# balisujohn/tortoise.cpp

Hardware: AMD Instinct MI355X
Metric: audio-seconds/sec end-to-end (AR+diffusion+vocoder), 16 cands x 80 steps (higher is better)
Workload: dtype f16 MFMA inputs / f32 accumulate (diffusion, vocoder convs); f32 weights, f16 KV (AR)

## Files before the change

### include/tortoise_mi355x.h

```cpp
#ifndef TORTOISE_MI355X_H
#define TORTOISE_MI355X_H

#include <stdint.h>

#ifdef __cplusplus
extern "C" {
#endif

typedef struct tts_ctx tts_ctx;

typedef enum {
  TTS_OK = 0,
  TTS_ERR_ARG = -1,
  TTS_ERR_IO = -2,
  TTS_ERR_FORMAT = -3,
  TTS_ERR_HIP = -4,
  TTS_ERR_STATE = -5,
  TTS_ERR_LIMIT = -6
} tts_status;

enum { TTS_VOCAB_MEL = 8194, TTS_DMODEL = 1024, TTS_MEL_CH = 100, TTS_CODES = 502 };

#define TTS_API_VERSION 8
int tts_version(void);
// ... 78 lines not shown
int tts_cvvp_latent_dim(const tts_ctx *ctx);
int tts_cvvp_rows(int mel_frames);
int tts_cvvp_voice(tts_ctx *ctx, const float *mel80, const int32_t *frames, int n_clips, float *latents_out);
int tts_cvvp_voice_audio(tts_ctx *ctx, const float *audio, const int64_t *n_samples, const int32_t *sample_rate, int n_clips, const tts_voice_audio_opts *opts,
                         float *latents_out);
int tts_cvvp_score(tts_ctx *ctx, const float *voice_latents, int n_clips, const int32_t *codes, const int32_t *code_len, int n_candidates, int code_stride,
                   float *scores_out);

int tts_diffusion_frames(int latent_rows);

int tts_load_hifigan(tts_ctx *ctx, const char *path);
int tts_hifigan_samples(int latent_rows);
#define TTS_HFG_HALO_FRAMES 24
int tts_hifigan_decode(tts_ctx *ctx, const float *latents, const int32_t *rows, int n_candidates, const float *voices, int n_voices,
                       const int32_t *voice_of_candidate, float *audio_out);
int tts_hifigan_chunk(tts_ctx *ctx, const float *latents, const int32_t *rows, int n_candidates, const float *voices, int n_voices,
                      const int32_t *voice_of_candidate, const int32_t *frame0, const int32_t *n_frames, float *audio_out);
typedef int (*tts_audio_cb)(void *user, const float *samples, int n_samples, int is_last);
int tts_hifigan_stream(tts_ctx *ctx, const int32_t *text_ids, int n_text, const float *voice1024, int max_steps, unsigned flags, int stride_codes,
                       tts_audio_cb cb, void *user, int32_t *codes_out , int32_t *rows_out, float *latents_out , int32_t *steps_out);
int tts_hifigan_stream_recaptures(const tts_ctx *ctx);
int tts_ar_session_open(tts_ctx *ctx, int n_slots, int max_cand, int max_text, int max_steps, unsigned flags);
int tts_ar_session_admit(tts_ctx *ctx, const int32_t *text_ids, int n_text, const float *voice1024, int n_cand, uint32_t seed,
                         const int32_t *stop_at );
int tts_ar_session_room(const tts_ctx *ctx);
int tts_ar_session_step(tts_ctx *ctx);
int tts_ar_session_finished(tts_ctx *ctx, int32_t *ids_out, int cap);
int tts_ar_session_collect(tts_ctx *ctx, int request, int32_t *codes_out , int32_t *rows_out, float *latents_out ,
                           int32_t *steps_out, int32_t *stopped_out );
int tts_ar_session_logits(tts_ctx *ctx, int request, float *logits_out );
int tts_ar_session_cancel(tts_ctx *ctx, int request);
int tts_ar_session_close(tts_ctx *ctx);
int tts_ar_session_recaptures(const tts_ctx *ctx);
int tts_ar_session_enable_audio(tts_ctx *ctx, int stride_steps);
int tts_ar_session_audio(tts_ctx *ctx, int request, float *out, int cap_samples, int32_t *is_last);
enum { TTS_AR_ROW_CONTROLS = 8 };
typedef struct tts_ar_request {
  uint32_t struct_size;
  int32_t n_cand;
  uint32_t seed;
  int32_t max_steps;
  const int32_t *stop_at;
  double temperature, top_k, top_p, repetition_penalty, penalty_scope;
  double typical_mass;
} tts_ar_request;
int tts_ar_request_init(tts_ctx *ctx, tts_ar_request *req);
int tts_ar_session_admit_ex(tts_ctx *ctx, const int32_t *text_ids, int n_text, const float *voice1024, const tts_ar_request *req);
int tts_host_ar_request_check(const tts_ar_request *req, int max_cand, int max_steps);
int tts_host_session_first_fit(const uint8_t *busy, int n_slots, int n_cand);
typedef struct tts_diff_request {
  uint32_t struct_size;
  int32_t n_cand;
  const float *latents;
  const int32_t *rows;
  const float *voice_latent2048;
  int32_t n_steps;
  int32_t sampler;
  double ddim_eta, cond_free_k;
  const float *noise;
  uint32_t seed;
  double temperature;
  int32_t cond_free;
} tts_diff_request;
int tts_diff_request_init(tts_ctx *ctx, tts_diff_request *req);
int tts_diff_session_open(tts_ctx *ctx, int max_packed_rows, int max_requests);
int tts_diff_session_admit(tts_ctx *ctx, const tts_diff_request *req);
int tts_diff_session_room(const tts_ctx *ctx);
int tts_diff_session_step(tts_ctx *ctx);
int tts_diff_session_finished(tts_ctx *ctx, int32_t *ids, int cap);
int tts_diff_session_collect(tts_ctx *ctx, int request, float *mel_out);
int tts_diff_session_cancel(tts_ctx *ctx, int request);
int tts_diff_session_close(tts_ctx *ctx);
int tts_diff_session_captures(const tts_ctx *ctx);
int tts_host_diff_packed_rows(const int32_t *latent_rows, int n_cand);
int tts_host_diff_packed_rows_ex(const int32_t *latent_rows, int n_cand, int cond_free);
int tts_host_diff_request_check(const tts_diff_request *req, int max_packed_rows);
int tts_diffusion_forward(tts_ctx *ctx, const float *latents, int latent_rows, const float *x_t,
                          int timestep, int conditioning_free, float *out);
enum { TTS_NOISE_REFERENCE = 0, TTS_NOISE_DEVICE = 1 };
int tts_diffusion(tts_ctx *ctx, const float *latents, const int32_t *rows, int n_candidates,
                  int n_steps, const float *noise, int noise_mode, float *mel_out);
int tts_diffusion_last_layout(const tts_ctx *ctx, int32_t *packed_rows_out, int32_t *sequences_out);
int tts_diffusion_time_mlp_retries(const tts_ctx *ctx);
int tts_diffusion_fp16_check(tts_ctx *ctx, int64_t counts[2]);

int tts_vocoder_samples(int mel_frames);
int tts_vocoder(tts_ctx *ctx, const float *mel, const int32_t *frames, int n_candidates,
                const float *noise, int noise_mode, float *audio_out);

int tts_vocoder_chunk(tts_ctx *ctx, const float *mel, int mel_frames, const float *noise, int frame0, int n_frames,
                      float *audio_out, int *n_samples_out);

int tts_load_bigvgan(tts_ctx *ctx, const char *path);
int tts_bigvgan_samples(int mel_frames);
int tts_bigvgan(tts_ctx *ctx, const float *mel, const int32_t *frames, int n_candidates, float *audio_out);
int tts_bigvgan_config(tts_ctx *ctx, int32_t out[8]);

#define TTS_CLS_MAX_SAMPLES 220000
int tts_load_classifier(tts_ctx *ctx, const char *path);
int tts_classifier_positions(int n_samples_24k);
int tts_classify_audio(tts_ctx *ctx, const float *audio, const int64_t *n_samples, const int32_t *sample_rate, int n_clips, float *prob_out,
                       float *logits_out);

int tts_load_aligner(tts_ctx *ctx, const char *path);
int tts_aligner_frames(int n_samples_16k);
int tts_aligner_clip_frames(tts_ctx *ctx, int64_t n_samples, int sample_rate);
int tts_aligner_vocab(tts_ctx *ctx, int32_t *vocab_out, int cap, int32_t *blank_out);
int tts_aligner_ids(tts_ctx *ctx, const float *audio, const int64_t *n_samples, const int32_t *sample_rate, int n_clips, int32_t *ids_out,
                    int32_t *n_frames_out, int frame_stride, float *logits_out);
int tts_align_audio(tts_ctx *ctx, const float *audio, int64_t n_samples, int sample_rate, const char *text, int64_t *offsets_out, int cap);
int64_t tts_redact_audio(tts_ctx *ctx, const float *audio, int64_t n_samples, int sample_rate, const char *text, float *out, int64_t cap);
int tts_host_ctc_decode(const int32_t *ids, int n_frames, const int32_t *vocab, int n_vocab, int blank, char *out, int cap);
int tts_host_max_alignment(const char *s1, const char *s2, char *out, int cap);
int tts_host_ctc_align(const int32_t *ids, int n_frames, const int32_t *vocab, int n_vocab, int blank, const char *text, int64_t n_samples,
                       int64_t *offsets_out, int cap);
int tts_host_redact_spans(const char *text, char *clean_out, int cap, int32_t *intervals_out, int cap_intervals);

#define TTS_RANDOM_VOICE_MAX 4096
enum { TTS_RANDOM_VOICE_AUTO = 0, TTS_RANDOM_VOICE_DIFFUSION = 1 };
int tts_load_random_voice(tts_ctx *ctx, const char *auto_path, const char *diff_path);
int tts_random_voice_dim(const tts_ctx *ctx, int side);
int tts_random_voice(tts_ctx *ctx, const uint64_t *seeds, int n, const float *z_auto, const float *z_diff, float *out_auto, float *out_diff);
int tts_random_voice_noise(tts_ctx *ctx, uint64_t seed, int side, float *out, int cap);
int tts_host_blend_voices(const float *latents, const float *weights, int n, int dim, float *out);
int tts_host_random_voice_fold(const float *w, const float *b, int dim, int equal, float *w_out, float *b_out);

#define TTS_DVAE_MAX_CLIPS 256
#define TTS_DVAE_MAX_FRAMES 16384
int tts_load_dvae(tts_ctx *ctx, const char *path);
int tts_dvae_rows(int mel_frames);
int tts_dvae_tokens(const tts_ctx *ctx);
int tts_dvae_dim(const tts_ctx *ctx);
int tts_dvae_codes(tts_ctx *ctx, const float *mel80, const int32_t *frames, int n_clips, int32_t *codes_out, int32_t *n_codes_out, int code_stride,
                   float *z_out);
int tts_dvae_codes_audio(tts_ctx *ctx, const float *audio, const int64_t *n_samples, const int32_t *sample_rate, int n_clips,
                         const tts_voice_audio_opts *opts, int32_t *codes_out, int32_t *n_codes_out, int code_stride, float *z_out);
int tts_ar_latents_for_codes(tts_ctx *ctx, const int32_t *text_ids, int n_text, const float *voice1024, const int32_t *codes, int n_codes,
                             int32_t *rows_out, float *latents_out);

#define TTS_SCORE_POS_DECODE 0
#define TTS_SCORE_POS_TRAIN 1
int tts_ar_score_codes(tts_ctx *ctx, const int32_t *text_ids, int n_text, const float *voice1024, const int32_t *codes, const int32_t *n_codes, int n_cand,
                       int code_stride, int positions, float *logp_out, float *stop_logp_out, int32_t *greedy_out, float *lse_out);
int tts_host_ar_score_rows(const int32_t *codes, int n_codes, int positions, int32_t *input_ids, int32_t *mel_pos, int32_t *targets);

int tts_write_wav(const char *path, const float *samples, int64_t n, int sample_rate);

int tts_host_schedule_ddim(int n_steps, double eta, double *acp, double *acp_prev, float *c_x0, float *c_eps, float *sigma);
int tts_host_schedule_dpmpp(int n_steps, float *a, float *b, float *c, int32_t *order);
int tts_host_schedule(int n_steps, int32_t *timestep_map, float *max_log, float *min_log, float *cfk, float *sqrt_recip,
                      float *sqrt_recipm1, float *coef1, float *coef2);
void tts_host_timestep_embedding(int t, float *out1024);
int tts_host_rel_bucket(int query, int key);
int tts_host_sample_row(const float *row8194, const int32_t *penalty_ids, int n_ids, float uniform);
int tts_host_sample_prefiltered(const float *row8194, const int32_t *penalty_ids, int n_ids, float uniform, int keep);
int tts_host_sample_row_ex(const float *row8194, const int32_t *penalty_ids, int n_ids, float uniform, float temperature, int top_k, float top_p, float penalty,
                           int mode);
int tts_host_sample_prefiltered_ex(const float *row8194, const int32_t *penalty_ids, int n_ids, float uniform, float temperature, int top_k, float top_p,
                                   float penalty, int keep, int already_penalised);
int tts_host_typical_keep(const float *row8194, double mass, uint8_t *keep_out8194);
int tts_host_sample_row_typical(const float *row8194, const int32_t *penalty_ids, int n_ids, float uniform, float temperature, int top_k, float top_p,
                                float penalty, double typical_mass, int mode);
int tts_host_sample_prefiltered_typical(const float *row8194, const int32_t *penalty_ids, int n_ids, float uniform, float temperature, int top_k, float top_p,
                                        float penalty, double typical_mass, int keep);
int tts_host_pad_codes(const int32_t *codes, int n, int32_t *out502);
int tts_host_stream_final_rows(const int32_t *codes, int k);
// ... 16 lines not shown
```

### tortoise.cpp_amd/__init__.py

```python
import ctypes as C
import os
import subprocess
import numpy as np

HERE = os.path.dirname(os.path.abspath(__file__))
LIB_PATH = os.environ.get("TTS_LIB_PATH") or os.path.join(HERE, "libtortoise_mi355x.so")
HEADER = os.path.join(os.path.dirname(HERE), "include", "tortoise_mi355x.h")
VOCAB_MEL = 8194
DMODEL = 1024
AR_MASK_STOP = 1
AR_RETIRE = 2
AR_ROW_CONTROLS = 8
NOISE_REFERENCE, NOISE_DEVICE = 0, 1
SAMPLER_DDPM, SAMPLER_DDIM, SAMPLER_DPMPP_2M = 0, 1, 3
SCORE_POSITIONS = {"decode": 0, "train": 1}

_f32p = np.ctypeslib.ndpointer(np.float32, flags="C_CONTIGUOUS")
_i32p = np.ctypeslib.ndpointer(np.int32, flags="C_CONTIGUOUS")
_f64p = np.ctypeslib.ndpointer(np.float64, flags="C_CONTIGUOUS")
AUDIO_CB = C.CFUNCTYPE(C.c_int, C.c_void_p, C.POINTER(C.c_float), C.c_int, C.c_int)


def build(verbose=False):
    subprocess.check_call(["make", "-C", HERE, "-j8", "all"], stdout=None if verbose else subprocess.DEVNULL)


class ArRequest(C.Structure):
    _fields_ = [("struct_size", C.c_uint32), ("n_cand", C.c_int32), ("seed", C.c_uint32), ("max_steps", C.c_int32), ("stop_at", C.c_void_p),
                ("temperature", C.c_double), ("top_k", C.c_double), ("top_p", C.c_double), ("repetition_penalty", C.c_double), ("penalty_scope", C.c_double),
                ("typical_mass", C.c_double)]


AR_REQUEST_SIZE_V0 = ArRequest.typical_mass.offset


class DiffRequest(C.Structure):
    _fields_ = [("struct_size", C.c_uint32), ("n_cand", C.c_int32), ("latents", C.c_void_p), ("rows", C.c_void_p), ("voice_latent2048", C.c_void_p),
                ("n_steps", C.c_int32), ("sampler", C.c_int32), ("ddim_eta", C.c_double), ("cond_free_k", C.c_double), ("noise", C.c_void_p), ("seed", C.c_uint32),
                ("temperature", C.c_double), ("cond_free", C.c_int32)]


class VoiceAudioOpts(C.Structure):
    _fields_ = [("struct_size", C.c_uint32), ("mel_norms80", C.c_void_p), ("crop_offset", C.c_int64), ("full_clips", C.c_int32)]


AR_CONTROL_FIELDS = {"temperature": "temperature", "top_k": "top_k", "top_p": "top_p", "penalty": "repetition_penalty", "scope": "penalty_scope",
                     "typical_mass": "typical_mass"}


class TtsError(RuntimeError):
    pass


_lib = None


def lib():
    global _lib
    if _lib is not None:
        return _lib
    if not os.path.exists(LIB_PATH):
        raise TtsError("libtortoise_mi355x.so is not built (run __graft_entry__.build()); there is no fallback path")
    L = C.CDLL(LIB_PATH)
    vp, ci, cf = C.c_void_p, C.c_int, C.c_float
    sig = {
        "tts_version": (ci, []), "tts_create": (vp, [ci]), "tts_destroy": (None, [vp]), "tts_last_error": (C.c_char_p, [vp]),
        "tts_set_option": (ci, [vp, C.c_char_p, C.c_double]),
        "tts_load_ar": (ci, [vp, C.c_char_p]), "tts_load_diffusion": (ci, [vp, C.c_char_p]),
        "tts_load_vocoder": (ci, [vp, C.c_char_p]), "tts_load_clvp": (ci, [vp, C.c_char_p]),
        "tts_load_diffusion_conditioning_encoder": (ci, [vp, C.c_char_p]), "tts_diffusion_conditioning_latent": (ci, [vp, _f32p, _i32p, ci, _f32p]),
        "tts_set_diffusion_conditioning_latent": (ci, [vp, _f32p]),
        "tts_load_voice_encoder": (ci, [vp, C.c_char_p]), "tts_voice_latent": (ci, [vp, _f32p, _i32p, ci, _f32p]),
        "tts_load_cvvp": (ci, [vp, C.c_char_p]), "tts_cvvp_latent_dim": (ci, [vp]), "tts_cvvp_rows": (ci, [ci]),
        "tts_cvvp_voice": (ci, [vp, vp, vp, ci, vp]), "tts_cvvp_voice_audio": (ci, [vp, vp, vp, vp, ci, vp, vp]),
        "tts_cvvp_score": (ci, [vp, vp, ci, vp, vp, ci, ci, vp]),
        "tts_clvp_score": (ci, [vp, _i32p, ci, _i32p, _i32p, ci, ci, _f32p]), "tts_ar_layers": (ci, [vp]), "tts_diffusion_layers": (ci, [vp]),
        "tts_seed": (None, [vp, C.c_uint32]), "tts_rng_load_state": (ci, [vp, C.c_char_p]), "tts_rng_save_state": (ci, [vp, C.c_char_p]),
        "tts_rng_uniform": (cf, [vp]), "tts_rng_normal": (None, [vp, _f32p, C.c_int64]),
        "tts_tokenizer_load": (ci, [vp, C.c_char_p]), "tts_tokenize": (ci, [vp, C.c_char_p, _i32p, ci]),
        "tts_ar_begin": (ci, [vp, _i32p, ci, _f32p, ci, ci]), "tts_ar_prefill": (ci, [vp, _f32p]),
        "tts_ar_step": (ci, [vp, _i32p, ci, _f32p]), "tts_ar_latents": (ci, [vp, _i32p, ci, ci, _f32p]),
        "tts_sample": (ci, [vp, _f32p, _i32p, ci, ci, _i32p]),
        "tts_ar_step_sample": (ci, [vp, _i32p, ci, C.c_uint, _i32p]), "tts_ar_topk_fallbacks": (ci, [vp]), "tts_diffusion_time_mlp_retries": (ci, [vp]), "tts_diffusion_fp16_check": (ci, [vp, C.POINTER(C.c_int64)]),
        "tts_device_numa_node": (ci, [vp, C.c_char_p, ci]), "tts_pin_to_device_numa_node": (ci, [vp]),
        "tts_host_sample_row": (ci, [_f32p, _i32p, ci, cf]), "tts_host_sample_prefiltered": (ci, [_f32p, _i32p, ci, cf, ci]),
        "tts_host_sample_row_ex": (ci, [_f32p, _i32p, ci, cf, cf, ci, cf, cf, ci]), "tts_host_sample_prefiltered_ex": (ci, [_f32p, _i32p, ci, cf, cf, ci, cf, cf, ci, ci]),
        "tts_host_typical_keep": (ci, [_f32p, C.c_double, vp]),
        "tts_host_sample_row_typical": (ci, [_f32p, _i32p, ci, cf, cf, ci, cf, cf, C.c_double, ci]),
        "tts_host_sample_prefiltered_typical": (ci, [_f32p, _i32p, ci, cf, cf, ci, cf, cf, C.c_double, ci]),
        "tts_autoregressive": (ci, [vp, _i32p, ci, _f32p, ci, ci, C.c_uint, _i32p, _i32p, vp, _i32p]),
        "tts_ar_stop_status": (ci, [vp, _i32p, ci]), "tts_ar_set_stop_schedule": (ci, [vp, C.c_void_p, ci]),
        "tts_ar_begin_multi": (ci, [vp, _i32p, _i32p, ci, _f32p, _i32p, ci]),
        "tts_autoregressive_multi": (ci, [vp, _i32p, _i32p, ci, _f32p, _i32p, ci, C.c_uint, _i32p, _i32p, vp, _i32p]),
        "tts_split_text": (ci, [vp, C.c_char_p, ci, _i32p, _i32p, ci]),
        "tts_ar_begin_multi_voice": (ci, [vp, _i32p, _i32p, ci, vp, ci, vp, _i32p, ci]),
        "tts_autoregressive_multi_voice": (ci, [vp, _i32p, _i32p, ci, vp, ci, vp, _i32p, ci, C.c_uint, _i32p, _i32p, vp, _i32p]),
        "tts_diffusion_multi_voice": (ci, [vp, _f32p, _i32p, ci, vp, ci, vp, ci, vp, ci, _f32p]),
        "tts_split_turns": (ci, [vp, C.c_char_p, ci, ci, _i32p, _i32p, _i32p, ci]),
        "tts_host_ar_stop_run": (ci, [_i32p, ci, _i32p, ci, C.c_uint, vp, _i32p, _i32p, _i32p, vp]),
        "tts_diffusion_frames": (ci, [ci]),
        "tts_load_hifigan": (ci, [vp, C.c_char_p]), "tts_hifigan_samples": (ci, [ci]),
        "tts_hifigan_decode": (ci, [vp, vp, vp, ci, vp, ci, vp, vp]),
        "tts_hifigan_chunk": (ci, [vp, vp, vp, ci, vp, ci, vp, vp, vp, vp]),
        "tts_load_bigvgan": (ci, [vp, C.c_char_p]), "tts_bigvgan_samples": (ci, [ci]), "tts_bigvgan": (ci, [vp, vp, vp, ci, vp]),
        "tts_bigvgan_config": (ci, [vp, vp]),
        "tts_load_classifier": (ci, [vp, C.c_char_p]), "tts_classifier_positions": (ci, [ci]), "tts_classify_audio": (ci, [vp, vp, vp, vp, ci, vp, vp]),
        "tts_load_aligner": (ci, [vp, C.c_char_p]), "tts_aligner_frames": (ci, [ci]), "tts_aligner_clip_frames": (ci, [vp, C.c_int64, ci]),
        "tts_aligner_vocab": (ci, [vp, vp, ci, vp]), "tts_aligner_ids": (ci, [vp, vp, vp, vp, ci, vp, vp, ci, vp]),
        "tts_align_audio": (ci, [vp, vp, C.c_int64, ci, C.c_char_p, vp, ci]), "tts_redact_audio": (C.c_int64, [vp, vp, C.c_int64, ci, C.c_char_p, vp, C.c_int64]),
        "tts_host_ctc_decode": (ci, [vp, ci, vp, ci, ci, vp, ci]), "tts_host_max_alignment": (ci, [C.c_char_p, C.c_char_p, vp, ci]),
        "tts_host_ctc_align": (ci, [vp, ci, vp, ci, ci, C.c_char_p, C.c_int64, vp, ci]), "tts_host_redact_spans": (ci, [C.c_char_p, vp, ci, vp, ci]),
        "tts_load_random_voice": (ci, [vp, C.c_char_p, C.c_char_p]), "tts_random_voice_dim": (ci, [vp, ci]),
        "tts_random_voice": (ci, [vp, vp, ci, vp, vp, vp, vp]), "tts_random_voice_noise": (ci, [vp, C.c_uint64, ci, vp, ci]),
        "tts_load_dvae": (ci, [vp, C.c_char_p]), "tts_dvae_rows": (ci, [ci]), "tts_dvae_tokens": (ci, [vp]), "tts_dvae_dim": (ci, [vp]),
        "tts_dvae_codes": (ci, [vp, vp, vp, ci, vp, vp, ci, vp]), "tts_dvae_codes_audio": (ci, [vp, vp, vp, vp, ci, vp, vp, vp, ci, vp]),
        "tts_ar_latents_for_codes": (ci, [vp, vp, ci, vp, vp, ci, vp, vp]),
        "tts_ar_score_codes": (ci, [vp, vp, ci, vp, vp, vp, ci, ci, ci, vp, vp, vp, vp]), "tts_host_ar_score_rows": (ci, [vp, ci, ci, vp, vp, vp]),
        "tts_host_blend_voices": (ci, [vp, vp, ci, ci, vp]), "tts_host_random_voice_fold": (ci, [vp, vp, ci, ci, vp, vp]),
        "tts_hifigan_stream": (ci, [vp, vp, ci, vp, ci, C.c_uint, ci, vp, vp, vp, vp, vp, vp]), "tts_hifigan_stream_recaptures": (ci, [vp]),
        "tts_host_stream_final_rows": (ci, [vp, ci]),
        "tts_ar_session_open": (ci, [vp, ci, ci, ci, ci, C.c_uint]), "tts_ar_session_admit": (ci, [vp, vp, ci, vp, ci, C.c_uint32, vp]),
        "tts_ar_session_room": (ci, [vp]), "tts_ar_session_step": (ci, [vp]), "tts_ar_session_finished": (ci, [vp, vp, ci]),
        "tts_ar_session_collect": (ci, [vp, ci, vp, vp, vp, vp, vp]), "tts_ar_session_logits": (ci, [vp, ci, vp]),
        "tts_ar_session_cancel": (ci, [vp, ci]), "tts_ar_session_close": (ci, [vp]), "tts_ar_session_recaptures": (ci, [vp]),
        "tts_ar_session_enable_audio": (ci, [vp, ci]), "tts_ar_session_audio": (ci, [vp, ci, vp, ci, vp]),
        "tts_host_session_first_fit": (ci, [vp, ci, ci]),
        "tts_ar_request_init": (ci, [vp, C.POINTER(ArRequest)]), "tts_ar_session_admit_ex": (ci, [vp, vp, ci, vp, C.POINTER(ArRequest)]),
        "tts_host_ar_request_check": (ci, [C.POINTER(ArRequest), ci, ci]),
        "tts_diff_request_init": (ci, [vp, C.POINTER(DiffRequest)]), "tts_diff_session_open": (ci, [vp, ci, ci]),
        "tts_diff_session_admit": (ci, [vp, C.POINTER(DiffRequest)]), "tts_diff_session_room": (ci, [vp]), "tts_diff_session_step": (ci, [vp]),
        "tts_diff_session_finished": (ci, [vp, vp, ci]), "tts_diff_session_collect": (ci, [vp, ci, vp]), "tts_diff_session_cancel": (ci, [vp, ci]),
        "tts_diff_session_close": (ci, [vp]), "tts_diff_session_captures": (ci, [vp]),
        "tts_host_diff_packed_rows": (ci, [vp, ci]), "tts_host_diff_packed_rows_ex": (ci, [vp, ci, ci]),
        "tts_diffusion_last_layout": (ci, [vp, _i32p, _i32p]), "tts_host_diff_request_check": (ci, [C.POINTER(DiffRequest), ci]),
        "tts_diffusion_forward": (ci, [vp, _f32p, ci, _f32p, ci, ci, _f32p]),
        "tts_diffusion": (ci, [vp, _f32p, _i32p, ci, ci, vp, ci, _f32p]),
        "tts_vocoder_samples": (ci, [ci]),
        "tts_vocoder": (ci, [vp, _f32p, _i32p, ci, vp, ci, _f32p]),
        "tts_vocoder_chunk": (ci, [vp, _f32p, ci, _f32p, ci, ci, _f32p, C.POINTER(ci)]),
        "tts_write_wav": (ci, [C.c_char_p, _f32p, C.c_int64, ci]), "tts_read_wav": (C.c_int64, [C.c_char_p, vp, C.c_int64, vp]),
        "tts_voice_audio_opts_init": (ci, [C.POINTER(VoiceAudioOpts)]),
        "tts_voice_from_audio": (ci, [vp, vp, vp, vp, ci, vp, vp, vp]), "tts_audio_mel": (ci, [vp, vp, C.c_int64, ci, ci, vp, vp, C.c_int64]),
        "tts_host_schedule": (ci, [ci, _i32p] + [_f32p] * 7), "tts_host_schedule_ddim": (ci, [ci, C.c_double, _f64p, _f64p, _f32p, _f32p, _f32p]),
        "tts_host_schedule_dpmpp": (ci, [ci, _f32p, _f32p, _f32p, _i32p]), "tts_host_timestep_embedding": (None, [ci, _f32p]),
        "tts_host_rel_bucket": (ci, [ci, ci]), "tts_host_pad_codes": (ci, [_i32p, ci, _i32p]), "tts_host_trimmed_rows": (ci, [_i32p]),
        "tts_host_fp8_e4m3": (C.c_uint8, [cf]), "tts_host_mel_frames": (ci, [C.c_int64]),
        "tts_host_mel_diffusion100": (ci, [_f32p, C.c_int64, ci, _f32p]), "tts_host_mel_voice80": (ci, [_f32p, C.c_int64, vp, _f32p]),
        "tts_prof_reset": (ci, [vp, ci]), "tts_prof_get": (ci, [vp, C.c_char_p, C.POINTER(C.c_double), C.POINTER(C.c_int64), C.POINTER(C.c_double)]),
    }
    for name, (res, args) in sig.items():
        fn = getattr(L, name)
        fn.restype = res
        fn.argtypes = args
    _lib = L
    return L


def header_symbols():
    import re
    txt = open(HEADER).read()
    txt = re.sub(r"/\*.*?\*/", "", txt, flags=re.S)
    return sorted(set(re.findall(r"\b(tts_[a-z0-9_]+)\s*\(", txt)))


def _ptr(a):
    return None if a is None else a.ctypes.data_as(C.c_void_p)
# ... 34 lines not shown
    def set_option(self, key, value):
        self._ck(self.L.tts_set_option(self.h, key.encode(), float(value)))

    def load(self, model_dir=None, ar=None, diffusion=None, vocoder=None):
        if model_dir:
            ar = ar or os.path.join(model_dir, "ggml-model.bin")
            diffusion = diffusion or os.path.join(model_dir, "ggml-diffusion-model.bin")
            vocoder = vocoder or os.path.join(model_dir, "ggml-vocoder-model.bin")
        if ar:
            self._ck(self.L.tts_load_ar(self.h, ar.encode()))
        if diffusion:
            self._ck(self.L.tts_load_diffusion(self.h, diffusion.encode()))
        if vocoder:
            self._ck(self.L.tts_load_vocoder(self.h, vocoder.encode()))

    @property
    def ar_layers(self):
        return self.L.tts_ar_layers(self.h)

    def seed(self, s):
        self.L.tts_seed(self.h, s)

    def rng_load_state(self, path):
        self._ck(self.L.tts_rng_load_state(self.h, path.encode()))

    def rng_save_state(self, path):
        self._ck(self.L.tts_rng_save_state(self.h, path.encode()))

    def rng_uniform(self):
        return self.L.tts_rng_uniform(self.h)

    def rng_normal(self, n):
        out = np.empty(n, np.float32)
        self.L.tts_rng_normal(self.h, out, n)
        return out

    def tokenizer_load(self, path):
        return self._ck(self.L.tts_tokenizer_load(self.h, path.encode()))

    def tokenize(self, message):
        out = np.empty(4096, np.int32)
        n = self._ck(self.L.tts_tokenize(self.h, message.encode("utf-8"), out, 4096))
        return out[:n].copy()

    def ar_begin(self, tokens, voice, B, max_steps):
        self.B = B
        self._ck(self.L.tts_ar_begin(self.h, np.ascontiguousarray(tokens, np.int32), len(tokens),
                                     np.ascontiguousarray(voice, np.float32), B, max_steps))

    def ar_prefill(self):
        out = np.empty((self.B, VOCAB_MEL), np.float32)
        self._ck(self.L.tts_ar_prefill(self.h, out.reshape(-1)))
        return out

    def ar_step(self, prev_ids, i):
        out = np.empty((self.B, VOCAB_MEL), np.float32)
        self._ck(self.L.tts_ar_step(self.h, np.ascontiguousarray(prev_ids, np.int32), i, out.reshape(-1)))
        return out

    def ar_step_sample(self, prev_ids, i, mask_stop=False):
        out = np.empty(self.B, np.int32)
        self._ck(self.L.tts_ar_step_sample(self.h, np.ascontiguousarray(prev_ids, np.int32), i, 1 if mask_stop else 0, out))
        return out

    def topk_fallbacks(self):
        return self.L.tts_ar_topk_fallbacks(self.h)

    def numa_node(self):
        buf = C.create_string_buffer(1024)
        node = self.L.tts_device_numa_node(self.h, buf, 1024)
        return node, buf.value.decode()

    def pin_to_numa_node(self):
        return self.L.tts_pin_to_device_numa_node(self.h)

    def fp16_check(self):
        c = (C.c_int64 * 2)()
        self._ck(self.L.tts_diffusion_fp16_check(self.h, c))
        return int(c[0]), int(c[1])

    def time_mlp_retries(self):
        return self.L.tts_diffusion_time_mlp_retries(self.h)

    def ar_latents(self, codes502, n_mel=502):
        codes502 = np.ascontiguousarray(codes502, np.int32).reshape(-1, 502)
        nb = codes502.shape[0]
        out = np.empty((nb, min(500, n_mel), DMODEL), np.float32)
        self._ck(self.L.tts_ar_latents(self.h, codes502.reshape(-1), nb, n_mel, out.reshape(-1)))
        return out

    def sample(self, logits, penalty_ids):
        logits = np.ascontiguousarray(logits, np.float32)
        ids = np.ascontiguousarray(penalty_ids, np.int32).reshape(logits.shape[0], -1)
        out = np.empty(logits.shape[0], np.int32)
        self._ck(self.L.tts_sample(self.h, logits.reshape(-1), ids.reshape(-1), ids.shape[1], logits.shape[0], out))
        return out

    def set_stop_schedule(self, stop_at=None):
        if stop_at is None:
            self._ck(self.L.tts_ar_set_stop_schedule(self.h, None, 0))
        else:
            a = np.ascontiguousarray(stop_at, np.int32)
            self._ck(self.L.tts_ar_set_stop_schedule(self.h, a.ctypes.data_as(C.c_void_p), len(a)))

    def autoregressive(self, tokens, voice, B, max_steps, mask_stop=False, want_latents=True, retire=False):
        codes = np.empty((B, 502), np.int32)
        rows = np.empty(B, np.int32)
        steps = np.zeros(1, np.int32)
        lat = np.empty((B * 500, DMODEL), np.float32) if want_latents else None
        self._ck(self.L.tts_autoregressive(self.h, np.ascontiguousarray(tokens, np.int32), len(tokens),
                                           np.ascontiguousarray(voice, np.float32), B, max_steps,
                                           (AR_MASK_STOP if mask_stop else 0) | (AR_RETIRE if retire else 0), codes.reshape(-1), rows, _ptr(lat), steps))
        lats = None
        if want_latents:
            lats, off = [], 0
            for r in rows:
                lats.append(lat[off:off + r].copy())
                off += r
        return codes, rows, lats, int(steps[0])

    def ar_begin_multi(self, prompts, voice=None, n_cand=1, max_steps=1, voices=None, voice_of_prompt=None):
        ids, lens, nc = _prompt_args(prompts, n_cand)
        self.B = int(nc.sum())
        if voices is None and voice_of_prompt is None:
            self._ck(self.L.tts_ar_begin_multi(self.h, ids, lens, len(lens), np.ascontiguousarray(voice, np.float32), nc, max_steps))
            return
        tab, nv, idx = _voice_args(voice, voices, voice_of_prompt, DMODEL)
        self._ck(self.L.tts_ar_begin_multi_voice(self.h, ids, lens, len(lens), _ptr(tab), nv, _ptr(idx), nc, max_steps))

    def autoregressive_multi(self, prompts, voice=None, n_cand=1, max_steps=1, mask_stop=False, retire=False, want_latents=True, voices=None, voice_of_prompt=None):
        ids, lens, nc = _prompt_args(prompts, n_cand)
        B = int(nc.sum())
        codes = np.empty((B, 502), np.int32)
        rows = np.empty(B, np.int32)
        steps = np.zeros(1, np.int32)
        lat = np.empty((B * 500, DMODEL), np.float32) if want_latents else None
        flags = (AR_MASK_STOP if mask_stop else 0) | (AR_RETIRE if retire else 0)
        if voices is None and voice_of_prompt is None:
            self._ck(self.L.tts_autoregressive_multi(self.h, ids, lens, len(lens), np.ascontiguousarray(voice, np.float32), nc, max_steps, flags,
                                                     codes.reshape(-1), rows, _ptr(lat), steps))
        else:
            tab, nv, idx = _voice_args(voice, voices, voice_of_prompt, DMODEL)
            self._ck(self.L.tts_autoregressive_multi_voice(self.h, ids, lens, len(lens), _ptr(tab), nv, _ptr(idx), nc, max_steps, flags, codes.reshape(-1), rows,
                                                           _ptr(lat), steps))
        c0 = np.concatenate([[0], np.cumsum(nc)])
        out_codes = [codes[c0[g]:c0[g + 1]].copy() for g in range(len(nc))]
        out_rows = [rows[c0[g]:c0[g + 1]].copy() for g in range(len(nc))]
        out_lats = None
        if want_latents:
            out_lats, off = [], 0
            for g in range(len(nc)):
                lg = []
                for r in out_rows[g]:
                    lg.append(lat[off:off + r].copy())
                    off += r
                out_lats.append(lg)
        return out_codes, out_rows, out_lats, int(steps[0])

    def split_text(self, message, max_ids):
        raw = message.encode("utf-8")
        cap = len(raw) + 1
        starts, lens = np.empty(cap, np.int32), np.empty(cap, np.int32)
        n = self._ck(self.L.tts_split_text(self.h, raw, max_ids, starts, lens, cap))
        return [raw[starts[k]:starts[k] + lens[k]].decode("utf-8") for k in range(n)]

    def split_turns(self, message, n_voices, max_ids=404):
# ... 868 lines not shown
```

### tortoise.cpp_amd/csrc/api.cpp

```cpp
#include "common.h"
#include <sched.h>
#include <cctype>
#include <cstddef>
#include <cmath>
#include <algorithm>
#include <chrono>
#include <fstream>
#include <new>

using namespace tts;

hipEvent_t tts::prof_event(tts_ctx *c) {
  if (!c->ev_pool.empty()) { hipEvent_t e = c->ev_pool.back(); c->ev_pool.pop_back(); return e; }
  hipEvent_t e = nullptr;
  (void)hipEventCreate(&e);
  return e;
}

template <class F>
static int guarded(tts_ctx *c, F body) {
  try {
    return body();
  } catch (const std::bad_alloc &) {
    return fail(c, TTS_ERR_LIMIT, "out of host memory");
// ... 86 lines not shown
  diff_session_close(c);
  if (c->ar) ar_free(c->ar);
  if (c->diff) diff_free(c->diff);
  if (c->voc) voc_free(c->voc);
  if (c->clvp) clvp_free(c->clvp);
  if (c->cvvp) cvvp_free(c->cvvp);
  if (c->venc) voice_enc_free(c->venc);
  if (c->dcond) diff_cond_enc_free(c->dcond);
  if (c->hifigan) hifigan_free(c->hifigan);
  if (c->bigvgan) bigvgan_free(c->bigvgan);
  if (c->classifier) classifier_free(c->classifier);
  if (c->aligner) aligner_free(c->aligner);
  if (c->dvae) dvae_free(c->dvae);
  if (c->rlg) random_voice_free(c->rlg);
  if (c->afe) afe_free(c->afe);
  if (c->fp16_counts) (void)hipFree(c->fp16_counts);
  delete c->tok;
  for (auto &kv : c->prof)
    for (auto &pr : kv.second.pending) { (void)hipEventDestroy(pr.first); (void)hipEventDestroy(pr.second); }
  for (hipEvent_t e : c->ev_pool) (void)hipEventDestroy(e);
  if (c->ev0) (void)hipEventDestroy(c->ev0);
  if (c->ev1) (void)hipEventDestroy(c->ev1);
  if (c->stream) (void)hipStreamDestroy(c->stream);
  if (c->load_stream) (void)hipStreamDestroy(c->load_stream);
  delete c;
}

int tts_version(void) { return TTS_API_VERSION; }

const char *tts_last_error(const tts_ctx *c) { return c ? c->err.c_str() : "no context (no HIP device?)"; }

static const char *const kArControlKeys[6] = {"ar_temperature", "ar_top_k", "ar_top_p", "ar_repetition_penalty", "ar_penalty_scope", "ar_typical_mass"};
static int ar_control_index(const std::string &k) {
  for (int i = 0; i < 6; i++)
    if (k == kArControlKeys[i]) return i;
  return -1;
}
static const char *ar_control_error(int which, double value) {
  static_assert(TTS_VOCAB_MEL == 8194, "the text below names the vocabulary size");
  switch (which) {
  case 0: return (!std::isfinite(value) || !(value > 0) || !std::isfinite((float)value) || !((float)value > 0)) ? "ar_temperature: a finite value > 0" : nullptr;
  case 1: return (!(value >= 1 && value <= TTS_VOCAB_MEL) || value != std::floor(value)) ? "ar_top_k: an integer in 1 .. 8194" : nullptr;
  case 2: return (!(value > 0 && value <= 1) || !((float)value > 0)) ? "ar_top_p: a value in (0, 1]" : nullptr;
  case 3: return (!std::isfinite(value) || !(value >= 1) || !std::isfinite((float)value)) ? "ar_repetition_penalty: a finite value >= 1" : nullptr;
  case 4: return (value != 0 && value != 1) ? "ar_penalty_scope: 0 (the ids of the last input) or 1 (every id fed since tts_ar_begin)" : nullptr;
  case 5: return (value != 0 && (!(value > 0 && value < 1) || !((float)value > 0 && (float)value < 1))) ? "ar_typical_mass: 0 (off) or a value in (0, 1)" : nullptr;
  }
  return "unknown sampler control";
}
static void ar_control_store(int which, double value, SamplerParams &sp, int &scope) {
  switch (which) {
  case 0: sp.temp = (float)value; break;
  case 1: sp.top_k = (int)value; break;
  case 2: sp.top_p = (float)value; break;
  case 3: sp.penalty = (float)value; break;
  case 4: scope = (int)value; break;
  case 5: sp.typ_mass = (float)value; break;
  }
}

int tts_set_option(tts_ctx *c, const char *key, double value) {
  if (!c || !key) return TTS_ERR_ARG;
  std::string k(key);
  if (k == "gn_eps") c->gn_eps = (float)value;
  else if (k == "ggml_lut") c->ggml_lut = value != 0;
  else if (k.rfind("prof_only:", 0) == 0) {
    if (value != 0) c->prof_filter.push_back(k.substr(10));
    else c->prof_filter.clear();
  }
  else if (k == "device_topk") c->device_topk = value != 0;
  else if (k == "sampler_threads") {
    if (c->sampler_pool) { sampler_pool_free(c->sampler_pool); c->sampler_pool = nullptr; }
    c->sampler_threads = value < 0 ? -1 : (int)value;
  }
  else if (k == "share_uncond") c->share_uncond = value != 0;
  else if (k == "prof_stride") c->prof_stride = value < 1 ? 1 : (int)value;
  else if (k == "diff_graph") c->diff_graph = value != 0;
  else if (k == "dec_f32_mfma") c->dec_f32_mfma = value != 0;
  else if (k == "attn_f32") c->attn_f32 = value != 0;
  else if (k == "attn_proj_f16") c->attn_proj_f16 = value != 0;
  else if (k == "proj_dual_b") c->proj_dual_b = value != 0;
  else if (k == "gemm_wreg") c->gemm_wreg = value == 1 ? tts_ctx::GEMM_WREG_ALL : value == 2 ? 1 : value == 3 ? 2 : value == 4 ? 4 : 0;
  else if (k == "gemm_gn_fuse") c->gemm_gn_fuse = value != 0;
  else if (k == "lc_attn_f32") c->lc_attn_f32 = value != 0;
  else if (k == "latency_mode") c->latency_mode = value != 0;
  else if (k == "fp16_check") c->fp16_check = value != 0;
  else if (k == "rng_fast_normal") c->rng_fast_normal = value != 0;
  else if (k == "noise_pipeline") c->noise_pipeline = value != 0;
  else if (k == "load_device_pack") c->load_device_pack = value != 0;
  else if (k == "load_threads") c->load_threads = value < 0 ? 0 : value > 64 ? 64 : (int)value;
  else if (k == "attn_q64") c->attn_q64 = value < 0 ? 0 : value > 2 ? 2 : (int)value;
  else if (k == "hoist_integrator") c->hoist_integrator = value < 0 ? 0 : (int)value;
  else if (k == "attn_f32_drop") c->attn_f32_drop = (int)value & 7;
  else if (k == "ar_weights") {
    if (value != 0 && value != 1 && value != 2) return fail(c, TTS_ERR_ARG, "ar_weights: 0 (f32), 1 (fp16) or 2 (fp8 e4m3)");
    c->ar_weights = (int)value;
  }
  else if (k == "diff_sampler") {
    if (const char *e = diff_control_error(0, value)) return fail(c, TTS_ERR_ARG, "%s", e);
    c->diff_sampler = (int)value;
  }
  else if (k == "ddim_eta") {
    if (const char *e = diff_control_error(1, value)) return fail(c, TTS_ERR_ARG, "%s", e);
    c->ddim_eta = value;
  }
  else if (k == "cond_free_k") {
    if (const char *e = diff_control_error(2, value)) return fail(c, TTS_ERR_ARG, "%s", e);
    c->cond_free_k = (float)value;
  }
  else if (k == "diff_temperature") {
    if (const char *e = diff_control_error(3, value)) return fail(c, TTS_ERR_ARG, "%s", e);
    c->diff_temperature = value;
  }
  else if (k == "cond_free") {
    if (const char *e = diff_control_error(4, value)) return fail(c, TTS_ERR_ARG, "%s", e);
    c->cond_free = (int)value;
  }
  else if (ar_control_index(k) >= 0) {
    const int which = ar_control_index(k);
    if (const char *e = ar_control_error(which, value)) return fail(c, TTS_ERR_ARG, "%s", e);
    ar_control_store(which, value, c->ar_sp, c->ar_penalty_scope);
  }
  else if (k == "hfg_small_m") {
    if (!(value >= 0 && value <= (1 << 24)) || value != std::floor(value)) return fail(c, TTS_ERR_ARG, "hfg_small_m: a row count in 0 .. 2^24 (0 = never)");
    c->hfg_small_m = (int)value;
  }
  else if (k == "prof_eager_every") c->prof_eager_every = value < 1 ? 1 : (int)value;
  else if (k == "stream_cus") {
    if (c->device < 0) return fail(c, TTS_ERR_HIP, "host-only context: no stream");
    if (c->ar || c->diff || c->voc || c->clvp || c->cvvp || c->venc || c->dcond || c->hifigan) return fail(c, TTS_ERR_STATE, "stream_cus must be set before the models are loaded");
    (void)hipSetDevice(c->device);
    hipDeviceProp_t prop;
    if (hipGetDeviceProperties(&prop, c->device) != hipSuccess) return fail(c, TTS_ERR_HIP, "hipGetDeviceProperties failed");
    const int xcds = 8, per_xcd = prop.multiProcessorCount / xcds, n = (int)(value < 0 ? -value : value);
    if (prop.multiProcessorCount % xcds || per_xcd > 32 || n >= per_xcd) return fail(c, TTS_ERR_ARG, "stream_cus %d: the device has %d CUs per XCD", (int)value, per_xcd);
    hipStream_t s = nullptr;
    if (n == 0) {
      if (hipStreamCreate(&s) != hipSuccess) return fail(c, TTS_ERR_HIP, "hipStreamCreate failed");
    } else {
      uint32_t mask[8] = {0, 0, 0, 0, 0, 0, 0, 0};
      for (int slot = 0; slot < per_xcd; slot++)
        if ((slot < n) == (value > 0))
          for (int x = 0; x < xcds; x++) { const int bit = slot * xcds + x; mask[bit >> 5] |= 1u << (bit & 31); }
      if (hipExtStreamCreateWithCUMask(&s, (uint32_t)((per_xcd * xcds + 31) / 32), mask) != hipSuccess)
        return fail(c, TTS_ERR_HIP, "hipExtStreamCreateWithCUMask failed");
    }
    (void)hipStreamSynchronize(c->stream);
    (void)hipStreamDestroy(c->stream);
    c->stream = s;
    c->stream_cus = (int)value;
  }
  else if (k == "rng_shard_offset") { if (value < 0) return fail(c, TTS_ERR_ARG, "rng_shard_offset < 0"); c->rng_shard_offset = (int)value; }
  else if (k == "rng_shard_total") { if (value < 0) return fail(c, TTS_ERR_ARG, "rng_shard_total < 0"); c->rng_shard_total = (int)value; }
  else return fail(c, TTS_ERR_ARG, "unknown option '%s'", key);
  return TTS_OK;
}

#define NEED_CTX(c)                                                                              \
  do {                                                                                         \
    if (!(c)) return TTS_ERR_ARG;                                                              \
    if ((c)->device < 0) return fail((c), TTS_ERR_HIP, "host-only context: no HIP device, no CPU fallback"); \
    (void)hipSetDevice((c)->device);                                                           \
  } while (0)

#define NO_SESSION(c, name)                                                                                          \
  do {                                                                                                               \
// ... 271 lines not shown
    for (int b = 0; b < n_cand; b++)
      for (int j = 0; j <= n_codes[b]; j++) {
        const size_t r = (size_t)b * n_rows + j;
        if (lse_out) lse_out[b * os + j] = out[r];
        logp_out[b * os + j] = out[R + r];
        if (stop_logp_out) stop_logp_out[b * os + j] = out[2 * R + r];
        if (greedy_out) memcpy(&greedy_out[b * os + j], &out[3 * R + r], 4);
      }
    return TTS_OK;
  });
}
int tts_host_stream_final_rows(const int32_t *codes, int k) { return (k < 0 || (k > 0 && !codes)) ? TTS_ERR_ARG : stream_final_rows(codes, k); }
int tts_ar_layers(const tts_ctx *c) { return c ? ar_layers(c) : 0; }
int tts_diffusion_layers(const tts_ctx *c) { return c ? diff_layers(c) : 0; }

void tts_seed(tts_ctx *c, uint32_t seed) {
  if (!c) return;
  c->seed_value = seed;
  c->generator.seed(seed);
  c->distribution.reset();
  c->normal_distribution.reset();
}
int tts_rng_load_state(tts_ctx *c, const char *path) {
  if (!c) return TTS_ERR_ARG;
  std::ifstream fin(path);
  if (!fin) return fail(c, TTS_ERR_IO, "cannot open '%s'", path);
  fin >> c->generator;
  c->distribution.reset();
  c->normal_distribution.reset();
  return fin ? TTS_OK : fail(c, TTS_ERR_FORMAT, "bad RNG state file '%s'", path);
}
int tts_rng_save_state(tts_ctx *c, const char *path) {
  if (!c || !path) return TTS_ERR_ARG;
  std::ofstream fout(path);
  if (!fout) return fail(c, TTS_ERR_IO, "cannot open '%s' for writing", path);
  fout << c->generator;
  return fout ? TTS_OK : fail(c, TTS_ERR_IO, "cannot write '%s'", path);
}
float tts_rng_uniform(tts_ctx *c) { return c ? c->distribution(c->generator) : 0.f; }
void tts_rng_normal(tts_ctx *c, float *out, int64_t n) {
  if (!c || !out || n <= 0) return;
  rng_normal_fill(c, out, n);
}

int tts_tokenizer_load(tts_ctx *c, const char *path) {
  if (!c || !path) return TTS_ERR_ARG;
  return guarded(c, [&] {
    std::unique_ptr<Tokenizer> t(new Tokenizer());
    if (!t->load(path)) return fail(c, TTS_ERR_IO, "Failed to open %s (missing, truncated or malformed)", path);
    delete c->tok;
    c->tok = t.release();
    return (int)c->tok->vocab.size();
  });
}
int tts_tokenize(tts_ctx *c, const char *message, int32_t *out, int cap) {
  if (!c || !c->tok) return c ? fail(c, TTS_ERR_STATE, "tokenizer not loaded") : TTS_ERR_ARG;
  if (!message || !out || cap < 0) return fail(c, TTS_ERR_ARG, "tts_tokenize: bad argument");
  return guarded(c, [&] {
    std::vector<int> ids = c->tok->encode(message);
    for (int i = 0; i < (int)ids.size() && i < cap; i++) out[i] = ids[i];
    return (int)ids.size();
  });
}

int tts_ar_begin(tts_ctx *c, const int32_t *ids, int n, const float *voice, int B, int max_steps) {
  NEED_CTX(c);
  NO_SESSION(c, "tts_ar_begin");
  return guarded(c, [&] { return ar_begin(c, ids, n, voice, B, max_steps); });
}
int tts_ar_prefill(tts_ctx *c, float *logits) { NEED_CTX(c); NO_SESSION(c, "tts_ar_prefill"); return guarded(c, [&] { return ar_prefill(c, logits); }); }
int tts_ar_step(tts_ctx *c, const int32_t *prev, int i, float *logits) {
  NEED_CTX(c);
  NO_SESSION(c, "tts_ar_step");
  return guarded(c, [&] { return ar_step(c, prev, i, logits, 0); });
}
int tts_ar_step_sample(tts_ctx *c, const int32_t *prev, int i, unsigned flags, int32_t *samples_out) {
  NEED_CTX(c);
  NO_SESSION(c, "tts_ar_step_sample");
  if (!prev || !samples_out) return TTS_ERR_ARG;
  return guarded(c, [&] { return ar_drv_step_sample(c, prev, i, flags, samples_out); });
}
int tts_ar_topk_fallbacks(const tts_ctx *c) { return c ? c->topk_fallbacks : -1; }
int tts_diffusion_time_mlp_retries(const tts_ctx *c) { return c ? c->time_mlp_retries : -1; }
int tts_diffusion_fp16_check(tts_ctx *c, int64_t counts[2]) {
  if (!c || !counts) return TTS_ERR_ARG;
  return guarded(c, [&] { return tts::diff_fp16_check(c, counts); });
}
int tts_host_sample_row(const float *row, const int32_t *ids, int ids_per_cand, float uniform) {
  if (!row || !ids || ids_per_cand < 1) return -1;
  return sample_one_row(row, ids, ids_per_cand, uniform);
}
static bool sampler_params_ok(const float *row, const int32_t *ids, int n_ids, float temperature, int top_k, float top_p, float penalty) {
  if (!row || n_ids < 0 || (n_ids > 0 && !ids)) return false;
  for (int i = 0; i < n_ids; i++)
    if (ids[i] < 0 || ids[i] >= TTS_VOCAB_MEL) return false;
  return std::isfinite(temperature) && temperature > 0 && top_k >= 1 && top_k <= TTS_VOCAB_MEL && top_p > 0 && top_p <= 1 && std::isfinite(penalty) && penalty >= 1;
}
int tts_host_sample_row_ex(const float *row, const int32_t *ids, int n_ids, float uniform, float temperature, int top_k, float top_p, float penalty, int mode) {
  if (!sampler_params_ok(row, ids, n_ids, temperature, top_k, top_p, penalty) || (mode != 0 && mode != 1)) return -2;
  SamplerParams sp; sp.temp = temperature; sp.top_k = top_k; sp.top_p = top_p; sp.penalty = penalty;
  return sample_one_row_ex(row, ids, n_ids, uniform, sp, mode == 1);
}
int tts_host_sample_prefiltered_ex(const float *row, const int32_t *ids, int n_ids, float uniform, float temperature, int top_k, float top_p, float penalty, int keep,
                                   int already_penalised) {
  if (!sampler_params_ok(row, ids, n_ids, temperature, top_k, top_p, penalty) || keep < 1 || keep > TTS_PF_MAX) return -2;
  SamplerParams sp; sp.temp = temperature; sp.top_k = top_k; sp.top_p = top_p; sp.penalty = penalty;
  std::vector<int32_t> list(TTS_PF_WORDS);
  std::vector<float> pen;
  if (already_penalised) {
    pen.assign(row, row + TTS_VOCAB_MEL);
    for (int i = 0; i < n_ids; i++) { const float g = row[ids[i]]; pen[ids[i]] = g < 0 ? g * penalty : g / penalty; }
    row = pen.data();
  }
  if (host_prefilter_row(row, keep, list.data()) < 0) return -1;
  return sample_one_from_list_ex(list.data(), ids, n_ids, uniform, sp, already_penalised != 0);
}
int tts_host_typical_keep(const float *row, double mass, uint8_t *keep_out) {
  if (!row || !keep_out || mass == 0 || ar_control_error(5, mass)) return -2;
  return typical_keep(row, (double)(float)mass, (char *)keep_out);
}
int tts_host_sample_row_typical(const float *row, const int32_t *ids, int n_ids, float uniform, float temperature, int top_k, float top_p, float penalty, double mass,
                                int mode) {
  if (!sampler_params_ok(row, ids, n_ids, temperature, top_k, top_p, penalty) || (mode != 0 && mode != 1) || ar_control_error(5, mass)) return -2;
  SamplerParams sp; sp.temp = temperature; sp.top_k = top_k; sp.top_p = top_p; sp.penalty = penalty; sp.typ_mass = (float)mass;
  return sample_one_row_ex(row, ids, n_ids, uniform, sp, mode == 1);
}
int tts_host_sample_prefiltered_typical(const float *row, const int32_t *ids, int n_ids, float uniform, float temperature, int top_k, float top_p, float penalty,
                                        double mass, int keep) {
  if (ar_control_error(5, mass)) return -2;
  if (mass == 0) return tts_host_sample_prefiltered_ex(row, ids, n_ids, uniform, temperature, top_k, top_p, penalty, keep, 1);
  if (!sampler_params_ok(row, ids, n_ids, temperature, top_k, top_p, penalty) || keep < 1 || keep > TTS_PF_MAX) return -2;
  SamplerParams sp; sp.temp = temperature; sp.top_k = top_k; sp.top_p = top_p; sp.penalty = penalty; sp.typ_mass = (float)mass;
  std::vector<int32_t> list(TTS_PF_WORDS);
  std::vector<float> pen(row, row + TTS_VOCAB_MEL);
  for (int i = 0; i < n_ids; i++) { const float g = row[ids[i]]; pen[ids[i]] = g < 0 ? g * penalty : g / penalty; }
  if (host_prefilter_row_typical(pen.data(), (double)sp.typ_mass, keep, list.data()) < 0) return -1;
  return sample_one_from_list_ex(list.data(), ids, n_ids, uniform, sp, true);
}
int tts_host_sample_prefiltered(const float *row, const int32_t *ids, int ids_per_cand, float uniform, int keep) {
  if (!row || !ids || ids_per_cand < 1 || keep < 1 || keep > TTS_PF_MAX) return -2;
  std::vector<int32_t> list(TTS_PF_WORDS);
  if (host_prefilter_row(row, keep, list.data()) < 0) return -1;
  return sample_one_from_list(list.data(), ids, ids_per_cand, uniform);
}
int tts_ar_latents(tts_ctx *c, const int32_t *codes, int nb, int n_mel, float *out) {
  NEED_CTX(c);
  NO_SESSION(c, "tts_ar_latents");
  return guarded(c, [&] { return ar_latents(c, codes, nb, n_mel, out); });
}
int tts_sample(tts_ctx *c, const float *logits, const int32_t *ids, int ids_per_cand, int B, int32_t *out) {
  if (!c || !logits || !ids || !out || B < 1 || ids_per_cand < 1) return TTS_ERR_ARG;
  for (int i = 0; i < B * ids_per_cand; i++)
    if (ids[i] < 0 || ids[i] >= TTS_VOCAB_MEL) return fail(c, TTS_ERR_ARG, "penalty id out of range");
  if (int rc = shard_check(c, B)) return rc;
  return guarded(c, [&] { sample_candidates(c, c->generator, c->ar_sp, logits, ids, ids_per_cand, B, out); return (int)TTS_OK; });
}

int tts_autoregressive(tts_ctx *c, const int32_t *text_ids, int n_text, const float *voice, int B, int max_steps,
                       unsigned flags, int32_t *codes_out, int32_t *rows_out, float *latents_out, int32_t *steps_out) {
  NEED_CTX(c);
  NO_SESSION(c, "tts_autoregressive");
  return guarded(c, [&] {
    return ar_drv_autoregressive(c, text_ids, &n_text, 1, voice, 1, nullptr, &B, max_steps, flags, codes_out, rows_out, latents_out, steps_out);
  });
}

// ... 422 lines not shown
```

### tortoise.cpp_amd/csrc/common.h

```cpp
#pragma once
#include "../../include/tortoise_mi355x.h"
#include <hip/hip_runtime.h>
#include <cstdarg>
#include <cstdint>
#include <cstdio>
#include <cstring>
#include <functional>
#include <map>
#include <memory>
#include <random>
#include <algorithm>
#include <atomic>
#include <condition_variable>
#include <mutex>
#include <new>
#include <string>
#include <thread>
#include <vector>

namespace tts {

struct HostTensor {
  std::vector<float> data;
  int64_t ne[4] = {1, 1, 1, 1};
// ... 35 lines not shown
  void *p = nullptr;
  size_t cap = 0;
  ~PinnedBuf() { if (p) (void)hipHostFree(p); }
  PinnedBuf() = default;
  PinnedBuf(const PinnedBuf &) = delete;
  PinnedBuf &operator=(const PinnedBuf &) = delete;
  hipError_t reserve(size_t bytes) {
    if (bytes <= cap) return hipSuccess;
    if (p) (void)hipHostFree(p);
    p = nullptr; cap = 0;
    hipError_t e = hipHostMalloc(&p, bytes, hipHostMallocDefault);
    if (e == hipSuccess) cap = bytes;
    return e;
  }
  template <class T> T *as() const { return (T *)p; }
};

struct ProfEntry { double ms = 0, work = 0; int64_t launches = 0, seen = 0; std::vector<std::pair<hipEvent_t, hipEvent_t>> pending; };

struct ArState;
struct DiffState;
struct VocState;
struct ClvpState;
struct CvvpState;
struct VoiceEncState;
struct DiffCondEncState;
struct HifiganState;
struct BigvganState;
struct ClassifierState;
struct AlignerState;
struct DvaeState;
struct RandomVoiceState;
struct AfeState;
struct Tokenizer;
struct SamplerPool;
void sampler_pool_free(SamplerPool *p);
struct ArSession;
struct DiffSession;
struct ArExtendItem { int slot, n_text, have, upto; const int32_t *codes502; };
struct SamplerParams {
  float temp = 0.8f;
  int top_k = 50;
  float top_p = 0.8f;
  float penalty = 2.0f;
  double top_p_cut() const { return 1.0 - (double)top_p; }
  float typ_mass = 0.f;
};

}

struct tts_ctx {
  int device = 0;
  hipStream_t stream = nullptr;
  hipStream_t load_stream = nullptr;
  int stream_cus = 0;
  std::string err;
  float gn_eps = 1e-6f;
  int ggml_lut = 0;
  std::mt19937 generator;
  std::uniform_real_distribution<float> distribution{0.0, 1.0};
  std::normal_distribution<double> normal_distribution{0.0, 1.0};
  uint32_t seed_value = 0;
  tts::ArState *ar = nullptr;
  tts::DiffState *diff = nullptr;
  tts::VocState *voc = nullptr;
  tts::ClvpState *clvp = nullptr;
  tts::CvvpState *cvvp = nullptr;
  tts::VoiceEncState *venc = nullptr;
  tts::DiffCondEncState *dcond = nullptr;
  tts::HifiganState *hifigan = nullptr;
  tts::BigvganState *bigvgan = nullptr;
  tts::ClassifierState *classifier = nullptr;
  tts::AlignerState *aligner = nullptr;
  tts::DvaeState *dvae = nullptr;
  tts::RandomVoiceState *rlg = nullptr;
  tts::AfeState *afe = nullptr;
  tts::Tokenizer *tok = nullptr;
  tts::ArSession *session = nullptr;
  tts::DiffSession *diff_session = nullptr;
  tts::SamplerPool *sampler_pool = nullptr;
  tts::SamplerParams ar_sp;
  int ar_penalty_scope = 0;
  int device_topk = 1;
  int time_mlp_retries = 0;
  int topk_fallbacks = 0;
  int sampler_threads = -1;
  bool share_uncond = true;
  int rng_shard_offset = 0, rng_shard_total = 0;
  std::vector<int32_t> stop_schedule;
  std::vector<int32_t> ar_stopped;
  bool prof_on = false;
  std::vector<std::string> prof_filter;
  int prof_stride = 1;
  int ar_weights = 0;
  int dec_f32_mfma = 0;
  int attn_f32 = 0;
  static constexpr int GEMM_WREG_ALL = 7;
  int gemm_wreg = GEMM_WREG_ALL;
  int gemm_gn_fuse = 1;
  int proj_dual_b = 1;
  int attn_f32_drop = 0;
  int lc_attn_f32 = 1;
  int attn_proj_f16 = 0;
  int fp16_check = 0;
  int64_t fp16_bad_weights[2] = {0, 0};
  void *fp16_counts = nullptr;
  int rng_fast_normal = 1;
  int noise_pipeline = 1;
  int load_device_pack = 1;
  int load_threads = 0;
  int attn_q64 = 0;
  int hoist_integrator = 1;
  int latency_mode = 0;
  int diff_sampler = 0;
  double ddim_eta = 0;
  float cond_free_k = 2.0f;
  int cond_free = 1;
  double diff_temperature = 1.0;
  int last_diff_rows = -1, last_diff_seqs = 0;
  bool capturing = false;
  int stream_recaptures = 0;
  int hfg_small_m = 0;
  int diff_graph = 1;
  int prof_eager_every = 8;
  std::map<std::string, tts::ProfEntry> prof;
  std::vector<hipEvent_t> ev_pool;
  hipEvent_t ev0 = nullptr, ev1 = nullptr;
};

namespace tts {

int fail(tts_ctx *ctx, int code, const char *fmt, ...);

void rng_normal_fill(tts_ctx *ctx, float *dst, int64_t n);

struct PinnedPool {
  explicit PinnedPool(size_t min_cap_ = (size_t)18 << 20, int max_bufs_ = 4) : min_cap(min_cap_), max_bufs(max_bufs_) {}
  size_t min_cap;
  int max_bufs, made = 0;
  std::mutex mu;
  std::condition_variable cv;
  std::vector<std::pair<void *, size_t>> idle;
  ~PinnedPool() { for (auto &b : idle) (void)hipHostFree(b.first); }
  std::pair<void *, size_t> take(size_t n) {
    std::unique_lock<std::mutex> lk(mu);
    for (;;) {
      for (size_t i = 0; i < idle.size(); i++)
        if (idle[i].second >= n) { auto b = idle[i]; idle.erase(idle.begin() + (long)i); return b; }
      if (made < max_bufs) { made++; break; }
      if (!idle.empty()) { (void)hipHostFree(idle.back().first); idle.pop_back(); break; }
      cv.wait(lk);
    }
    lk.unlock();
    const size_t cap = std::max(n, min_cap);
    void *p = nullptr;
    if (hipHostMalloc(&p, cap, hipHostMallocDefault) != hipSuccess) {
      lk.lock(); made--; lk.unlock(); cv.notify_one();
      return {nullptr, 0};
    }
    return {p, cap};
  }
  void give(std::pair<void *, size_t> b) {
    if (!b.first) return;
    { std::lock_guard<std::mutex> lk(mu); idle.push_back(b); }
    cv.notify_one();
  }
  static hipError_t copy_now(void *dst, const void *src, size_t bytes, hipStream_t s) {
    if (!s) return hipMemcpy(dst, src, bytes, hipMemcpyHostToDevice);
    const hipError_t e = hipMemcpyAsync(dst, src, bytes, hipMemcpyHostToDevice, s);
    return e != hipSuccess ? e : hipStreamSynchronize(s);
  }
  hipError_t upload(void *dst, const void *src, size_t bytes, hipStream_t s = nullptr) {
    auto b = take(bytes);
    if (!b.first) return copy_now(dst, src, bytes, s);
    memcpy(b.first, src, bytes);
    const hipError_t e = copy_now(dst, b.first, bytes, s);
    give(b);
    return e;
  }
};

// ... 307 lines not shown
```

### tortoise.cpp_amd/csrc/diffusion.hip

```cpp
#include "common.h"
#include "gemm_f16.h"
#include <algorithm>
#include <chrono>
#include <cmath>

namespace tts {

static constexpr int C = 1024, NHEAD = 16, XTC = 128 ;
static constexpr int LAT_MAX_ROWS = 2048;
static constexpr int HOIST_MAX_ROWS = 16384;

__device__ __forceinline__ float silu_dev(float x, int lut) {
  if (lut == 1) {
    float xr = __half2float(__float2half_rn(x));
    return __half2float(__float2half_rn(xr / (1.0f + expf(-xr))));
  }
  if (lut == 2) return x / (1.0f + expf(-x));
  return x * __builtin_amdgcn_rcpf(1.0f + __builtin_amdgcn_exp2f(x * -1.44269504088896f));
}

__global__ __launch_bounds__(256) void gn_stats_kernel(const float *__restrict__ x, const int *__restrict__ seq_start,
                                                       const int *__restrict__ seq_len, float eps, float2 *__restrict__ stats) {
  __shared__ float sh[8];
  const int grp = blockIdx.x, s = blockIdx.y, T = seq_len[s];
// ... 657 lines not shown
  const DdimEntry *dtab;
  const DpmEntry *ptab;
  const __half *ce16_all;
  float *x;
  float *d_prev;
  const float *noise;
  unsigned long long seed;
  int n_steps, sampler, rows_local;
  unsigned stream_base;
  int guided;
};
__global__ __launch_bounds__(256) void step_begin_kernel(const ReqDev *__restrict__ req, const int *__restrict__ ctr, const int *__restrict__ live,
                                                         size_t ss_stride, float *__restrict__ ss_cur) {
  const int slot = live[blockIdx.y], k = ctr[slot];
  if (k >= req[slot].n_steps) return;
  const float4 *src = (const float4 *)(req[slot].ss_all + (size_t)k * ss_stride);
  float4 *dst = (float4 *)(ss_cur + (size_t)slot * ss_stride);
  for (size_t i = (size_t)blockIdx.x * 256 + threadIdx.x; i < ss_stride / 4; i += (size_t)gridDim.x * 256) dst[i] = src[i];
}
__global__ void step_advance_kernel(const ReqDev *__restrict__ req, int *__restrict__ ctr, const int *__restrict__ live, int n_live) {
  const int i = blockIdx.x * blockDim.x + threadIdx.x;
  if (i >= n_live) return;
  const int slot = live[i];
  if (ctr[slot] < req[slot].n_steps) ctr[slot] += 1;
}
__global__ __launch_bounds__(128) void step_xt_kernel(const ReqDev *__restrict__ req, const int *__restrict__ seq_req, const int64_t *__restrict__ seq_xoff,
                                                      const int *__restrict__ seq_partner, const int *__restrict__ row_seq, const int *__restrict__ row_t,
                                                      const int *__restrict__ seq_len, __half *__restrict__ xt16) {
  const int r = blockIdx.x, s = row_seq[r], ch = threadIdx.x;
  if (s < 0) return;
  const int p = seq_partner[s];
  if (p < 0) return;
  const int T = seq_len[s], t = row_t[r];
  const ReqDev &q = req[seq_req[s]];
  const float v = (ch < 100) ? q.x[seq_xoff[s] + (size_t)ch * T + t] : 0.f;
  const __half hv = __float2half_rn(v);
  xt16[(size_t)r * XTC + ch] = hv;
  if (q.guided) xt16[(size_t)(p + t) * XTC + ch] = hv;
}
__global__ __launch_bounds__(128) void step_row_select_kernel(const ReqDev *__restrict__ req, const int *__restrict__ ctr, const int *__restrict__ seq_req,
                                                              const int *__restrict__ row_seq, const int *__restrict__ row_src, uint4 *__restrict__ dst) {
  const int r = blockIdx.x, s = row_seq[r];
  uint4 v = make_uint4(0u, 0u, 0u, 0u);
  if (s >= 0) {
    const int slot = seq_req[s];
    const ReqDev &q = req[slot];
    const int k = min(ctr[slot], q.n_steps - 1);
    v = ((const uint4 *)(q.ce16_all + ((size_t)k * q.rows_local + row_src[r]) * C))[threadIdx.x];
  }
  dst[(size_t)r * (C / 8) + threadIdx.x] = v;
}
__global__ __launch_bounds__(128) void step_update_kernel(const float *__restrict__ net, const ReqDev *__restrict__ req, const int *__restrict__ ctr,
                                                          const int *__restrict__ seq_req, const int64_t *__restrict__ seq_xoff,
                                                          const int *__restrict__ seq_partner, const int *__restrict__ seq_cand,
                                                          const int *__restrict__ row_seq, const int *__restrict__ row_t, const int *__restrict__ seq_len) {
  const int r = blockIdx.x, s = row_seq[r], ch = threadIdx.x;
  if (s < 0 || ch >= 100) return;
  const int p = seq_partner[s];
  if (p < 0) return;
  const int slot = seq_req[s], k = ctr[slot];
  const ReqDev q = req[slot];
  if (k >= q.n_steps) return;
  const StepEntry e = q.tab[k];
  const float *noise = e.has_noise ? q.noise + e.noise_off : nullptr;
  const int T = seq_len[s], t = row_t[r];
  const size_t xi = seq_xoff[s] + (size_t)ch * T + t;
  const float eps_c = net[(size_t)r * 256 + ch];
  const bool guided = q.guided != 0;
  const float eps_u = guided ? net[(size_t)(p + t) * 256 + ch] : 0.f;
  const uint32_t stream = q.stream_base + (uint32_t)seq_cand[s], idx = (uint32_t)(ch * T + t);
  if (q.sampler == 1) {
    const DdimEntry d = q.dtab[k];
    q.x[xi] = ddim_step_value(e.sc, d, guided, eps_c, eps_u, q.x[xi], noise, xi, q.seed, stream, e.philox_step, idx);
  } else if (q.sampler == 3) {
    const DdimEntry d = q.dtab[k];
    const DpmEntry pe = q.ptab[k];
    q.x[xi] = dpmpp_step_value(e.sc, d, pe, guided, eps_c, eps_u, q.x[xi], q.d_prev, xi);
  } else {
    const float var_c = net[(size_t)r * 256 + 100 + ch];
    q.x[xi] = ddpm_step_value(e.sc, guided, eps_c, var_c, eps_u, q.x[xi], noise, xi, q.seed, stream, e.philox_step, idx);
  }
}

__global__ void philox_fill_kernel(float *__restrict__ x, int64_t n, uint64_t seed, uint32_t stream, uint32_t step) {
  int64_t i = (int64_t)blockIdx.x * blockDim.x + threadIdx.x;
  if (i < n) x[i] = philox_normal(seed, stream, step, (uint32_t)i);
}
__global__ void scale_xT_kernel(float *__restrict__ x, int64_t n, float temperature) {
  int64_t i = (int64_t)blockIdx.x * blockDim.x + threadIdx.x;
  if (i < n) x[i] = temperature * x[i];
}

__global__ void rows_to_ct_kernel(const float *__restrict__ net, int row0, int T, int nch, int ld, float *__restrict__ out) {
  int i = blockIdx.x * blockDim.x + threadIdx.x;
  if (i < nch * T) {
    int ch = i / T, t = i - ch * T;
    out[i] = net[(size_t)(row0 + t) * ld + ch];
  }
}

struct AttnDev {
  float *norm_g, *norm_b, *qkv_b, *proj_b, *bias_tab;
  __half *qkv_w, *proj_w;
  __half *qkv_wf;
  __half *proj_w_split;
  float proj_alpha;
};
struct ResDev { float *in_g, *in_b, *in_bias, *emb_w, *emb_b, *out_g, *out_b, *out_bias; __half *in_w, *out_w, *in_wf, *out_wf; };

struct Layout {
  int ns = 0, rows = 0;
  std::vector<int> start, len;
  DevBuf d_row_seq, d_row_t, d_start, d_len, d_chunk_seq;
  int build(tts_ctx *ctx, const std::vector<int> &lens) {
    has_seq_step = false; ss_step_stride = 0; gn_parts.clear();
    ns = (int)lens.size();
    len = lens;
    start.resize(ns);
    int r = 8;
    for (int s = 0; s < ns; s++) { start[s] = r; r = (r + lens[s] + 1 + 7) & ~7; }
    rows = (r + 127) & ~127;
    std::vector<int> rs(rows, -1), rt(rows, 0);
    for (int s = 0; s < ns; s++)
      for (int t = 0; t < lens[s]; t++) { rs[start[s] + t] = s; rt[start[s] + t] = t; }
    TTS_HIP(ctx, d_row_seq.reserve(rows * 4)); TTS_HIP(ctx, d_row_t.reserve(rows * 4));
    TTS_HIP(ctx, d_start.reserve(ns * 4)); TTS_HIP(ctx, d_len.reserve(ns * 4));
    TTS_HIP(ctx, hipMemcpy(d_row_seq.p, rs.data(), rows * 4, hipMemcpyHostToDevice));
    TTS_HIP(ctx, hipMemcpy(d_row_t.p, rt.data(), rows * 4, hipMemcpyHostToDevice));
    TTS_HIP(ctx, hipMemcpy(d_start.p, start.data(), ns * 4, hipMemcpyHostToDevice));
    TTS_HIP(ctx, hipMemcpy(d_len.p, len.data(), ns * 4, hipMemcpyHostToDevice));
    std::vector<int> cs(rows / 8, -1);
    for (int s = 0; s < ns; s++)
      for (int t = 0; t < lens[s]; t++) cs[(start[s] + t) >> 3] = s;
    TTS_HIP(ctx, d_chunk_seq.reserve(rows / 8 * 4));
    TTS_HIP(ctx, hipMemcpy(d_chunk_seq.p, cs.data(), rows / 8 * 4, hipMemcpyHostToDevice));
    return TTS_OK;
  }
  int max_len() const { return len.empty() ? 0 : *std::max_element(len.begin(), len.end()); }
  DevBuf d_seq_step;
  int ss_step_stride = 0;
  bool has_seq_step = false;
  const int *seq_step_ptr() const { return has_seq_step ? d_seq_step.as<int>() : nullptr; }
  struct GnPart { int s0, ns, row0, rows, tmax; };
  std::vector<GnPart> gn_parts;
  DevBuf d_start_rel;
  static int gn_class(int tmax) { return tmax <= 14 * 64 ? 0 : tmax <= 18 * 128 ? 1 : 2; }
  int set_gn_parts(tts_ctx *ctx, const std::vector<int> &cls_of_seq) {
    gn_parts.clear();
    std::vector<int> rel(ns, 0);
    for (int s = 0; s < ns;) {
      int e = s;
      while (e < ns && cls_of_seq[e] == cls_of_seq[s]) e++;
      GnPart g{s, e - s, s == 0 ? 0 : start[s], 0, 0};
      g.rows = (e < ns ? start[e] : rows) - g.row0;
      for (int i = s; i < e; i++) { rel[i] = start[i] - g.row0; g.tmax = std::max(g.tmax, len[i]); }
      gn_parts.push_back(g);
      s = e;
    }
    if (gn_parts.size() < 2) { gn_parts.clear(); return TTS_OK; }
    TTS_HIP(ctx, d_start_rel.reserve((size_t)ns * 4));
    TTS_HIP(ctx, hipMemcpy(d_start_rel.p, rel.data(), (size_t)ns * 4, hipMemcpyHostToDevice));
    return TTS_OK;
  }
  int set_seq_step(tts_ctx *ctx, const std::vector<int> &step_of_seq, int stride_floats) {
    TTS_HIP(ctx, d_seq_step.reserve(step_of_seq.size() * 4));
    TTS_HIP(ctx, hipMemcpy(d_seq_step.p, step_of_seq.data(), step_of_seq.size() * 4, hipMemcpyHostToDevice));
    ss_step_stride = stride_floats; has_seq_step = true;
    return TTS_OK;
  }
};

static hipError_t reserve_zeroed(DevBuf &b, size_t bytes) {
  const size_t old = b.cap;
  hipError_t e = b.reserve(bytes);
  if (e == hipSuccess && b.cap != old) e = hipMemset(b.p, 0, b.cap);
  return e;
}

struct Work {
  int rows = 0;
  DevBuf x, hbuf, a16, att16, qk16, vt16, stats;
  DevBuf att16_lo, qk16_lo, vt16_lo;
  long long *st_x = nullptr, *st_h = nullptr;
  float *X() { return x.as<float>(); }
  float *H() { return hbuf.as<float>(); }
  __half *A16() { return a16.as<__half>() + C; }
  __half *ATT16() { return att16.as<__half>() + C; }
  int reserve(tts_ctx *ctx, int r, int ns, bool split = false) {
    rows = r;
    TTS_HIP(ctx, reserve_zeroed(x, (size_t)r * C * 4));
    TTS_HIP(ctx, reserve_zeroed(hbuf, (size_t)r * C * 4));
    TTS_HIP(ctx, reserve_zeroed(a16, (size_t)(r + 2) * C * 2));
    TTS_HIP(ctx, reserve_zeroed(att16, (size_t)(r + 2) * C * 2));
    TTS_HIP(ctx, reserve_zeroed(qk16, (size_t)(r + 128) * 2048 * 2));
    TTS_HIP(ctx, reserve_zeroed(vt16, (size_t)C * (r + 128) * 2));
    TTS_HIP(ctx, reserve_zeroed(stats, (size_t)ns * 32 * sizeof(float2)));
    if (ctx->attn_f32 || split) {
      TTS_HIP(ctx, reserve_zeroed(att16_lo, (size_t)(r + 2) * C * 2));
      TTS_HIP(ctx, reserve_zeroed(qk16_lo, (size_t)(r + 128) * 2048 * 2));
      TTS_HIP(ctx, reserve_zeroed(vt16_lo, (size_t)C * (r + 128) * 2));
    }
    return TTS_OK;
  }
};

struct DiffReq {
  int n_cand = 0, n_steps = 0, sampler = 0;
  uint64_t seed = 0;
  uint32_t stream_base = 0;
  bool guided = true;
  int n_seq() const { return guided ? 2 * n_cand : n_cand; }
  bool host_noise = false;
  bool noise_streamed = false;
  int n_vec = 0;
  std::vector<int> T;
  std::vector<int64_t> xoff;
  int64_t total = 0;
  DevBuf ce16_all;
  DevBuf code_emb, h0;
  DevBuf ss_all, tab, dtab, ptab, x, d_prev, noise;
  std::chrono::steady_clock::time_point t_setup;
  int id = 0, slot = 0, done = 0, cls = 0, packed = 0;
  bool finished = false;
  std::vector<int> seq_src;
  int src_rows = 0;
  ReqDev dev() const {
    return ReqDev{ss_all.as<float>(), tab.as<StepEntry>(), dtab.as<DdimEntry>(), sampler == 3 ? ptab.as<DpmEntry>() : nullptr, ce16_all.as<__half>(), x.as<float>(),
                  sampler == 3 ? d_prev.as<float>() : nullptr, host_noise ? noise.as<float>() : nullptr, seed, n_steps, sampler, src_rows, stream_base, guided ? 1 : 0};
  }
};

struct StepBufs {
  Layout lay;
  Work wk;
  DevBuf code_emb, h0, ce, ce16, inp16, xt16, net;
  DevBuf ss_cur, ctr;
  DevBuf tables;
  const ReqDev *req = nullptr;
  const int64_t *seq_xoff = nullptr;
  const int *seq_req = nullptr, *seq_partner = nullptr, *seq_cand = nullptr, *row_src = nullptr, *live = nullptr;
  int n_live = 0;
  hipGraph_t step_graph = nullptr;
  hipGraphExec_t step_exec = nullptr;
  void drop_step_graph() {
    if (step_exec) (void)hipGraphExecDestroy(step_exec);
    if (step_graph) (void)hipGraphDestroy(step_graph);
    step_exec = nullptr; step_graph = nullptr;
  }
  ~StepBufs() { drop_step_graph(); }
  int reserve_rows(tts_ctx *ctx, size_t rows, bool integ) {
    TTS_HIP(ctx, reserve_zeroed(ce16, rows * C * 2));
    TTS_HIP(ctx, reserve_zeroed(inp16, rows * C * 2));
    TTS_HIP(ctx, reserve_zeroed(xt16, (rows + 2) * XTC * 2));
    TTS_HIP(ctx, reserve_zeroed(net, rows * 256 * 4));
    if (integ) {
      TTS_HIP(ctx, reserve_zeroed(code_emb, rows * C * 4));
      TTS_HIP(ctx, reserve_zeroed(ce, rows * C * 4));
    }
    return TTS_OK;
  }
  int set_tables(tts_ctx *ctx, const std::vector<ReqDev> &reqs, const std::vector<int> &slots, const std::vector<int64_t> &xoff, const std::vector<int> &sreq,
                 const std::vector<int> &partner, const std::vector<int> &cand, const std::vector<int> &rsrc) {
    std::vector<char> img;
    auto put = [&](const void *p, size_t bytes) { const size_t o = img.size(); img.insert(img.end(), (const char *)p, (const char *)p + bytes); return o; };
    const size_t o_req = put(reqs.data(), reqs.size() * sizeof(ReqDev)), o_xoff = put(xoff.data(), xoff.size() * 8);
    const size_t o_sreq = put(sreq.data(), sreq.size() * 4), o_partner = put(partner.data(), partner.size() * 4), o_cand = put(cand.data(), cand.size() * 4);
    const size_t o_rsrc = put(rsrc.data(), rsrc.size() * 4), o_live = put(slots.data(), slots.size() * 4);
    TTS_HIP(ctx, tables.reserve(img.size()));
    TTS_HIP(ctx, hipMemcpy(tables.p, img.data(), img.size(), hipMemcpyHostToDevice));
    const char *b = tables.as<char>();
    req = (const ReqDev *)(b + o_req); seq_xoff = (const int64_t *)(b + o_xoff);
    seq_req = (const int *)(b + o_sreq); seq_partner = (const int *)(b + o_partner); seq_cand = (const int *)(b + o_cand);
    row_src = (const int *)(b + o_rsrc); live = (const int *)(b + o_live);
    n_live = (int)slots.size();
    return TTS_OK;
  }
  int set_single(tts_ctx *ctx, const DiffReq &r) {
    const int B = r.n_cand;
    if (lay.ns != r.n_seq()) return fail(ctx, TTS_ERR_STATE, "diffusion step: a layout of %d sequences for a request of %d", lay.ns, r.n_seq());
    std::vector<int> sreq(lay.ns, 0), partner(lay.ns, -1), cand(lay.ns), rsrc(lay.rows, -1);
    std::vector<int64_t> xoff(lay.ns);
    for (int s = 0; s < lay.ns; s++) {
      cand[s] = s; xoff[s] = r.xoff[s % B];
      if (s < B) partner[s] = lay.start[r.guided ? s + B : s];
      for (int t = 0; t < lay.len[s]; t++) rsrc[lay.start[s] + t] = lay.start[s] + t;
    }
    return set_tables(ctx, {r.dev()}, {0}, xoff, sreq, partner, cand, rsrc);
  }
};

struct DiffState {
  int n_lc = 0, n_integ = 0, n_main = 0, n_tail = 0;
  std::vector<AttnDev> lc_attn, integ_attn, main_attn;
  std::vector<ResDev> integ_res, main_res, tail_res;
  float *cond_latent = nullptr, *uncond_emb = nullptr, *lc_bias = nullptr, *code_g = nullptr, *code_b = nullptr;
  float *te0_w = nullptr, *te0_b = nullptr, *te2_w = nullptr, *te2_b = nullptr;
  float *inp_bias = nullptr, *integ_bias = nullptr, *outn_g = nullptr, *outn_b = nullptr, *out_bias = nullptr;
  __half *lc_w = nullptr, *inp_w = nullptr, *integ_w = nullptr, *out_w = nullptr;
  std::vector<void *> owned;
  StepBufs sb;
  DiffReq req;
  Layout lat_lay, ilay;
  Work lat_wk, iwk;
  bool share_integ = false;
  DevBuf ce_src, iseq_src;
  bool hoisted = false;
  Layout play;
  Work pwk;
  DevBuf pcode, ph0, pce, psrc, pscatter;
  std::vector<int> ce_src_host;
  bool lat = false;
  DevBuf gn_stats, gn_stats_h0;
  int gn_site = 0, gn_sites_max = 0;
  size_t gn_slot_ll = 0, gn_stripe_ll = 0;
  long long *new_stats_slot() { long long *p = gn_stats.as<long long>() + (size_t)gn_site * gn_slot_ll; gn_site++; return p; }
  DevBuf temb, e1, emb, ss_chk, seq_src, lat_in16, out_ct;
  PinnedBuf noise_host;
  DevBuf mv_buf;
  const float *mv_tab = nullptr;
  const int *mv_idx = nullptr;
  ~DiffState() { for (void *p : owned) (void)hipFree(p); }
  int n_res() const { return n_integ + n_main + n_tail; }
};

void diff_free(DiffState *s) { delete s; }
int diff_layers(const tts_ctx *ctx) { return ctx->diff ? ctx->diff->n_main : 0; }
int diff_set_cond_latent(tts_ctx *ctx, const float *latent2048) {
  if (!ctx->diff) return fail(ctx, TTS_ERR_STATE, "tts_load_diffusion not called");
  if (!latent2048) return fail(ctx, TTS_ERR_ARG, "null latent");
  TTS_HIP(ctx, hipMemcpyAsync(ctx->diff->cond_latent, latent2048, (size_t)2 * C * 4, hipMemcpyHostToDevice, ctx->stream));
  TTS_HIP(ctx, hipStreamSynchronize(ctx->stream));
  return TTS_OK;
}

namespace {
struct Loader {
  tts_ctx *ctx; DiffState *st; const WeightFile &wf; std::map<std::string, bool> used; std::mutex mu; PinnedPool pin{(size_t)9 << 20, 4};
  const HostTensor *get(const std::string &name, int64_t nelem) {
    auto it = wf.t.find(name);
    if (it == wf.t.end()) { fail(ctx, TTS_ERR_FORMAT, "tensor '%s' missing from diffusion model file", name.c_str()); return nullptr; }
    if (it->second.nelem() != nelem) {
      fail(ctx, TTS_ERR_FORMAT, "tensor '%s' has wrong size in model file: got %lld, expected %lld", name.c_str(),
           (long long)it->second.nelem(), (long long)nelem);
      return nullptr;
    }
    { std::lock_guard<std::mutex> lk(mu); used[name] = true; }
    return &it->second;
  }
  template <class T> int put(const std::vector<T> &h, T **dst) {
    void *p = nullptr;
    TTS_HIP(ctx, hipMalloc(&p, h.size() * sizeof(T)));
    { std::lock_guard<std::mutex> lk(mu); st->owned.push_back(p); }
    TTS_HIP(ctx, pin.upload(p, h.data(), h.size() * sizeof(T), ctx->load_stream));
    *dst = (T *)p;
    return TTS_OK;
  }
  int f32(const std::string &name, int64_t n, float **dst) {
    const HostTensor *t = get(name, n);
    if (!t) return TTS_ERR_FORMAT;
    return put(t->data, dst);
  }
  int conv16(const std::string &name, int cout, int cin, int k, int cout_pad, int cin_pad, __half **dst, __half **dst_frag = nullptr) {
    const HostTensor *t = get(name, (int64_t)cout * cin * k);
    if (!t) return TTS_ERR_FORMAT;
    std::vector<__half> h((size_t)cout_pad * k * cin_pad, __float2half(0.f));
    const float *w = t->data.data();
    for (int co = 0; co < cout; co++)
      for (int ci = 0; ci < cin; ci++)
        for (int tap = 0; tap < k; tap++)
          h[(size_t)co * k * cin_pad + (size_t)tap * cin_pad + ci] = __float2half_rn(w[((size_t)co * cin + ci) * k + tap]);
    if (dst_frag) {
      std::vector<__half> f(h.size());
      for (int n = 0; n < cout_pad; n++)
        for (int tap = 0; tap < k; tap++)
          for (int c = 0; c < cin_pad; c++) f[gemm_wfrag3_index(n, tap, c, cout_pad, cin_pad)] = h[((size_t)n * k + tap) * cin_pad + c];
      if (int r = put(f, dst_frag)) return r;
    }
    return put(h, dst);
  }
  int attn(const std::string &p, AttnDev &a) {
    int r;
    if ((r = f32(p + ".norm.weight", C, &a.norm_g))) return r;
    if ((r = f32(p + ".norm.bias", C, &a.norm_b))) return r;
    if ((r = conv16(p + ".qkv.weight", 3 * C, C, 1, 3 * C, C, &a.qkv_w, &a.qkv_wf))) return r;
    if ((r = f32(p + ".qkv.bias", 3 * C, &a.qkv_b))) return r;
    if ((r = conv16(p + ".proj_out.weight", C, C, 1, C, C, &a.proj_w))) return r;
    {
      const HostTensor *t = get(p + ".proj_out.weight", (int64_t)C * C);
      std::vector<__half> sp((size_t)C * 2 * C);
      float amax = 0.f;
      for (float v : t->data) amax = std::max(amax, std::fabs(v));
      if (!std::isfinite(amax)) { fail(ctx, TTS_ERR_FORMAT, "tensor '%s.proj_out.weight' holds a non-finite value", p.c_str()); return TTS_ERR_FORMAT; }
      int e = 14;
      while (e > -14 && std::ldexp(amax, e) >= 30000.0f) e--;
      const float scale = std::ldexp(1.0f, e);
      a.proj_alpha = 1.0f / scale;
      for (int n = 0; n < C; n++)
        for (int k = 0; k < C; k++) {
          const float w = t->data[(size_t)n * C + k] * scale;
// ... 2 lines not shown
          sp[(size_t)n * 2 * C + C + k] = __float2half_rn(w - __half2float(hi));
        }
      long long bad[2] = {0, 0};
      for (const __half &h : sp) {
        const float v = std::fabs(__half2float(h));
        if (!(v <= 65504.0f)) bad[0]++;
        else if (v > 60000.0f) bad[1]++;
      }
      if (bad[0] | bad[1]) { std::lock_guard<std::mutex> lk(mu); ctx->fp16_bad_weights[0] += bad[0]; ctx->fp16_bad_weights[1] += bad[1]; }
      if ((r = put(sp, &a.proj_w_split))) return r;
    }
    if ((r = f32(p + ".proj_out.bias", C, &a.proj_b))) return r;
    const HostTensor *t = get(p + ".relative_pos_embeddings.relative_attention_bias.weight", 32 * 16);
    if (!t) return TTS_ERR_FORMAT;
    std::vector<float> tab(16 * 128);
    for (int h = 0; h < 16; h++)
      for (int sgn = 0; sgn < 2; sgn++)
        for (int d = 0; d < 64; d++) {
          int bucket = sgn ? rel_bucket(0, d) : rel_bucket(d, 0);
          if (d == 0) bucket = rel_bucket(0, 0);
          tab[h * 128 + sgn * 64 + d] = t->data[(size_t)bucket * 16 + h] * 8.0f;
        }
    return put(tab, &a.bias_tab);
  }
  int res(const std::string &p, ResDev &w) {
    int r;
    if ((r = f32(p + ".in_layers.0.weight", C, &w.in_g))) return r;
    if ((r = f32(p + ".in_layers.0.bias", C, &w.in_b))) return r;
    if ((r = conv16(p + ".in_layers.2.weight", C, C, 1, C, C, &w.in_w, &w.in_wf))) return r;
    if ((r = f32(p + ".in_layers.2.bias", C, &w.in_bias))) return r;
    if ((r = f32(p + ".emb_layers.1.weight", 2 * C * C, &w.emb_w))) return r;
    if ((r = f32(p + ".emb_layers.1.bias", 2 * C, &w.emb_b))) return r;
    if ((r = f32(p + ".out_layers.0.weight", C, &w.out_g))) return r;
    if ((r = f32(p + ".out_layers.0.bias", C, &w.out_b))) return r;
    if ((r = conv16(p + ".out_layers.3.weight", C, C, 3, C, C, &w.out_w, &w.out_wf))) return r;
    if ((r = f32(p + ".out_layers.3.bias", C, &w.out_bias))) return r;
    return TTS_OK;
  }
};
}

int diff_load(tts_ctx *ctx, const char *path) {
  ctx->fp16_bad_weights[0] = ctx->fp16_bad_weights[1] = 0;
  WeightFile wf;
  std::string err;
  int rc = read_weight_file(path, wf, err);
  if (rc != TTS_OK) return fail(ctx, rc, "diffusion_model_load: %s", err.c_str());
  std::unique_ptr<DiffState> st(new DiffState());
  Loader ld{ctx, st.get(), wf, {}};
  while (wf.has("latent_conditioner." + std::to_string(st->n_lc + 1) + ".norm.weight")) st->n_lc++;
  while (wf.has("conditioning_timestep_integrator." + std::to_string(st->n_integ) + ".resblk.in_layers.0.weight")) st->n_integ++;
  while (wf.has("layers." + std::to_string(st->n_main) + ".resblk.in_layers.0.weight")) st->n_main++;
  while (wf.has("layers." + std::to_string(st->n_main + st->n_tail) + ".in_layers.0.weight")) st->n_tail++;
  st->lc_attn.resize(st->n_lc);
  st->integ_res.resize(st->n_integ); st->integ_attn.resize(st->n_integ);
  st->main_res.resize(st->n_main); st->main_attn.resize(st->n_main);
  st->tail_res.resize(st->n_tail);
  std::vector<std::function<int()>> jobs;
  DiffState *S = st.get();
#define J(x) jobs.emplace_back([&ld, S]() -> int { (void)S; return (x); })
  J(ld.f32("diffusion_conditioning_latent", 2 * C, &S->cond_latent));
  J(ld.f32("unconditioned_embedding", C, &S->uncond_emb));
  J(ld.conv16("latent_conditioner.0.weight", C, C, 3, C, C, &S->lc_w));
  J(ld.f32("latent_conditioner.0.bias", C, &S->lc_bias));
  for (int i = 0; i < st->n_lc; i++) jobs.emplace_back([&ld, S, i]() { return ld.attn("latent_conditioner." + std::to_string(i + 1), S->lc_attn[i]); });
  J(ld.f32("code_norm.weight", C, &S->code_g));
  J(ld.f32("code_norm.bias", C, &S->code_b));
  J(ld.f32("time_embed.0.weight", C * C, &S->te0_w)); J(ld.f32("time_embed.0.bias", C, &S->te0_b));
  J(ld.f32("time_embed.2.weight", C * C, &S->te2_w)); J(ld.f32("time_embed.2.bias", C, &S->te2_b));
  for (int i = 0; i < st->n_integ; i++) {
    jobs.emplace_back([&ld, S, i]() { return ld.res("conditioning_timestep_integrator." + std::to_string(i) + ".resblk", S->integ_res[i]); });
    jobs.emplace_back([&ld, S, i]() { return ld.attn("conditioning_timestep_integrator." + std::to_string(i) + ".attn", S->integ_attn[i]); });
  }
  J(ld.conv16("inp_block.weight", C, 100, 3, C, XTC, &S->inp_w));
  J(ld.f32("inp_block.bias", C, &S->inp_bias));
  J(ld.conv16("integrating_conv.weight", C, 2 * C, 1, C, 2 * C, &S->integ_w));
  J(ld.f32("integrating_conv.bias", C, &S->integ_bias));
  for (int i = 0; i < st->n_main; i++) {
    jobs.emplace_back([&ld, S, i]() { return ld.res("layers." + std::to_string(i) + ".resblk", S->main_res[i]); });
    jobs.emplace_back([&ld, S, i]() { return ld.attn("layers." + std::to_string(i) + ".attn", S->main_attn[i]); });
  }
  for (int i = 0; i < st->n_tail; i++) jobs.emplace_back([&ld, S, i]() { return ld.res("layers." + std::to_string(S->n_main + i), S->tail_res[i]); });
  J(ld.f32("out.0.weight", C, &S->outn_g)); J(ld.f32("out.0.bias", C, &S->outn_b));
  J(ld.conv16("out.2.weight", 200, C, 3, 256, C, &S->out_w));
  jobs.emplace_back([&ld, S]() -> int {
    const HostTensor *t = ld.get("out.2.bias", 200);
    if (!t) return TTS_ERR_FORMAT;
    std::vector<float> b(256, 0.f);
    std::copy(t->data.begin(), t->data.end(), b.begin());
    return ld.put(b, &S->out_bias);
  });
#undef J
  if (int r = run_parallel(ctx, (int)jobs.size(), [&](int i) { return jobs[i](); })) return r;
  for (auto &kv : wf.t)
    if (!ld.used.count(kv.first)) return fail(ctx, TTS_ERR_FORMAT, "unknown tensor '%s' in model file", kv.first.c_str());
  TTS_HIP(ctx, hipFuncSetAttribute((const void *)diff_attn_f32_kernel, hipFuncAttributeMaxDynamicSharedMemorySize, ATT32_LDS));
  if (ctx->diff) diff_free(ctx->diff);
  ctx->diff = st.release();
  return TTS_OK;
}

#define CHECK(x) do { int _r = (x); if (_r) return _r; } while (0)

#ifdef TTS_DEBUG_CHECKSUM
static void dbg_sum(tts_ctx *ctx, const char *tag, const void *p, size_t bytes) {
  std::vector<uint8_t> h(bytes);
  (void)hipMemcpyAsync(h.data(), p, bytes, hipMemcpyDeviceToHost, ctx->stream);
  (void)hipStreamSynchronize(ctx->stream);
  uint64_t x = 1469598103934665603ull;
  for (size_t i = 0; i < bytes; i++) x = (x ^ h[i]) * 1099511628211ull;
  fprintf(stderr, "[cks] %s %016llx\n", tag, (unsigned long long)x);
  if (!strncmp(tag, "time", 4)) {
    static std::map<std::string, std::vector<float>> first;
    const float *f = (const float *)h.data();
    const size_t n = bytes / 4;
    auto it = first.find(tag);
    if (it == first.end()) first[tag].assign(f, f + n);
    else {
      size_t nd = 0, i0 = 0; float worst = 0.f;
      for (size_t i = 0; i < n; i++) if (memcmp(&f[i], &it->second[i], 4)) { if (!nd) i0 = i; nd++; worst = std::max(worst, fabsf(f[i] - it->second[i])); }
      if (nd) fprintf(stderr, "[dif] %s: %zu of %zu floats differ from the first call, first at %zu (%.9g vs %.9g), largest difference %.3g\n", tag, nd, n, i0, f[i0], it->second[i0], worst);
    }
  }
}
#define DBG_SUM(tag, p, bytes) dbg_sum(ctx, tag, p, bytes)
#else
#define DBG_SUM(tag, p, bytes)
#endif
static int fp16_check(tts_ctx *ctx, const void *p, size_t n_halves) {
  if (!ctx->fp16_check) return TTS_OK;
  if (!ctx->fp16_counts) {
    TTS_HIP(ctx, hipMalloc(&ctx->fp16_counts, 16));
    TTS_HIP(ctx, hipMemset(ctx->fp16_counts, 0, 16));
  }
  fp16_scan_kernel<<<512, 256, 0, ctx->stream>>>((const __half *)p, n_halves, (unsigned long long *)ctx->fp16_counts);
  TTS_HIP(ctx, hipGetLastError());
  return TTS_OK;
}
int diff_fp16_check(tts_ctx *ctx, int64_t counts[2]) {
  int64_t dev[2] = {0, 0};
  if (ctx->fp16_counts) {
    TTS_HIP(ctx, hipStreamSynchronize(ctx->stream));
    TTS_HIP(ctx, hipMemcpy(dev, ctx->fp16_counts, 16, hipMemcpyDeviceToHost));
  }
  counts[0] = dev[0] + ctx->fp16_bad_weights[0];
  counts[1] = dev[1] + ctx->fp16_bad_weights[1];
  return TTS_OK;
}

static int gemm(tts_ctx *ctx, const char *fam, GemmArgs &g, const Layout &lay, int n_valid = 0, int k_valid = 0) {
  double mv = 0;
  for (int l : lay.len) mv += l;
  static const bool log_shapes = getenv("TTS_GEMM_LOG") != nullptr;
  if (log_shapes) fprintf(stderr, "gemm M=%d N=%d K=%dx%d mode=%d resid=%d\n", g.M, g.N, g.nseg, g.kseg, g.mode, g.resid != nullptr);
  if (!strcmp(fam, "diff_gemm")) {
    if (g.mode == GEMM_OUT_QKV) fam = "diff_gemm_qkv";
    else if (gemm_is_conv3(g) && g.N == C && g.kseg == C) fam = g.resid ? "diff_gemm_k3r" : "diff_gemm_k3";
    else if (g.nseg == 1 && g.N == C && g.kseg == C && g.mode == GEMM_OUT_F32) fam = g.resid ? "diff_gemm_k1r" : "diff_gemm_k1";
    else if (g.custom_w && g.N == C && g.kseg == C && g.mode == GEMM_OUT_F32_SCALED && g.resid) fam = "diff_gemm_k1r";
    else fam = "diff_gemm_misc";
  }
  ProfScope ps(ctx, fam, 2.0 * mv * (n_valid ? n_valid : g.N) * (k_valid ? k_valid : g.nseg * g.kseg));
  TTS_HIP(ctx, launch_gemm_f16(g, ctx->stream));
  if (ctx->fp16_check) {
    if (gemm_mode_qkv(g.mode)) {
      CHECK(fp16_check(ctx, g.outH, (size_t)g.M * g.ldh));
      CHECK(fp16_check(ctx, g.outVt, (size_t)(g.N / 3) * g.ldvt));
// ... 372 lines not shown
    GemmArgs c3 = gemm_base(lay, wk.ATT16(), C, 3, C, w.out_w, C, w.out_bias);
    c3.Wf = w.out_wf; c3.wreg = gemm_wreg_class(ctx, 4);
    c3.mode = GEMM_OUT_F32; c3.outF = X; c3.ldo = C; c3.resid = xin;
    wk.st_x = nullptr;
    return gemm(ctx, "diff_gemm", c3, lay);
  }
  if (!Hpre) {
    long long *slot = lat ? st->new_stats_slot() : nullptr;
    CHECK(res_in_layers(ctx, st, lay, wk, xin, w, wk.H(), lat ? wk.st_x : nullptr, slot));
    Hpre = wk.H();
    st_h = slot;
  }
  DBG_SUM("res.out ss", ss, (size_t)2 * C * 4);
  DBG_SUM("res.out hpre", Hpre, (size_t)lay.rows * C * 4);
  CHECK(gn(ctx, st, lay, Hpre, lat ? st_h : nullptr, w.out_g, w.out_b, ss, 1, wk.A16(), lat ? w.out_w : gemm_wreg_image(ctx, 4, lay, C, w.out_w, w.out_wf), (size_t)3 * C * C * 2));
  DBG_SUM("res.out gn", wk.A16(), (size_t)lay.rows * C * 2);
  GemmArgs c3 = gemm_base(lay, wk.A16(), C, 3, C, w.out_w, C, w.out_bias);
  c3.Wf = w.out_wf; c3.wreg = gemm_wreg_class(ctx, 4);
  long long *st_out = lat ? st->new_stats_slot() : nullptr;
  c3.mode = st_out ? GEMM_OUT_F32_STATS : GEMM_OUT_F32; c3.outF = X; c3.ldo = C; c3.resid = xin;
  c3.st_out = st_out; c3.st_stripe_ll = (int)st->gn_stripe_ll; c3.chunk_seq = lay.d_chunk_seq.as<int>();
  wk.st_x = st_out;
  CHECK(gemm(ctx, "diff_gemm", c3, lay));
  DBG_SUM("res.out conv", X, (size_t)lay.rows * C * 4);
  return TTS_OK;
}

template <int CTRL> __device__ __forceinline__ float lnk_dpp(float x) {
  return __int_as_float(__builtin_amdgcn_update_dpp(0, __float_as_int(x), CTRL, 0xf, 0xf, false));
}
__device__ __forceinline__ float wave_sum_dpp(float x) {
  auto a = __builtin_amdgcn_permlane32_swap(__float_as_uint(x), __float_as_uint(x), false, false);
  x = __uint_as_float(a[0]) + __uint_as_float(a[1]);
  auto b = __builtin_amdgcn_permlane16_swap(__float_as_uint(x), __float_as_uint(x), false, false);
  x = __uint_as_float(b[0]) + __uint_as_float(b[1]);
  x += lnk_dpp<0x128>(x);
  x += lnk_dpp<0x124>(x);
  x += lnk_dpp<0x122>(x);
  x += lnk_dpp<0x121>(x);
  return x;
}

static constexpr int LNK_COLS = 32;
static __global__ __launch_bounds__(1024) void linear_nk_kernel(const float *__restrict__ x, int ldx, int rows, const float *__restrict__ W,
                                                         int N, const float *__restrict__ b, float *__restrict__ out, int ldo,
                                                         int act ) {
  const int lane = threadIdx.x & 63;
  for (int half = 0; half < 2; half++) {
    const int n = blockIdx.x * LNK_COLS + half * 16 + (threadIdx.x >> 6);
    if (n >= N) return;
    const float *wr = W + (size_t)n * C + lane * 4;
    float4 w[4];
#pragma unroll
    for (int j = 0; j < 4; j++) w[j] = *(const float4 *)(wr + j * 256);
    const float bn = b ? b[n] : 0.f;
    for (int r = 0; r < rows; r++) {
      const float *xr = x + (size_t)r * ldx + lane * 4;
      float acc = 0.f;
#pragma unroll
      for (int j = 0; j < 4; j++) {
        const float4 xv = *(const float4 *)(xr + j * 256);
        acc = fmaf(xv.x, w[j].x, acc); acc = fmaf(xv.y, w[j].y, acc);
        acc = fmaf(xv.z, w[j].z, acc); acc = fmaf(xv.w, w[j].w, acc);
      }
      float v = wave_sum_dpp(acc);
      if (lane == 0) {
        v += bn;
        if (act) {
          if (act == 2) v = __half2float(__float2half_rn(v));
          v = v / (1.f + expf(-v));
          if (act == 2) v = __half2float(__float2half_rn(v));
        }
        out[(size_t)r * ldo + n] = v;
      }
    }
  }
}

static __global__ __launch_bounds__(256) void differ_kernel(const unsigned *__restrict__ a, const unsigned *__restrict__ b, size_t n, int *__restrict__ flag) {
  for (size_t i = (size_t)blockIdx.x * 256 + threadIdx.x; i < n; i += (size_t)gridDim.x * 256)
    if (a[i] != b[i]) *flag = 1;
}

static int precompute_time(tts_ctx *ctx, DiffState *st, const std::vector<int> &timesteps, DevBuf &ss_all) {
  const int n = (int)timesteps.size(), nres = st->n_res();
  std::vector<float> te((size_t)n * C);
  for (int i = 0; i < n; i++) timestep_embedding(timesteps[i], te.data() + (size_t)i * C);
  TTS_HIP(ctx, st->temb.reserve(te.size() * 4)); TTS_HIP(ctx, st->e1.reserve(te.size() * 4)); TTS_HIP(ctx, st->emb.reserve(te.size() * 4));
  TTS_HIP(ctx, ss_all.reserve((size_t)n * nres * 2 * C * 4));
  TTS_HIP(ctx, hipMemcpyAsync(st->temb.p, te.data(), te.size() * 4, hipMemcpyHostToDevice, ctx->stream));
  TTS_HIP(ctx, hipStreamSynchronize(ctx->stream));
  const int act = ctx->ggml_lut ? 2 : 1;
  auto mlp = [&](float *ss_out) {
    linear_nk_kernel<<<C / LNK_COLS, 1024, 0, ctx->stream>>>(st->temb.as<float>(), C, n, st->te0_w, C, st->te0_b, st->e1.as<float>(), C, act);
    linear_nk_kernel<<<C / LNK_COLS, 1024, 0, ctx->stream>>>(st->e1.as<float>(), C, n, st->te2_w, C, st->te2_b, st->emb.as<float>(), C, act);
    for (int j = 0; j < nres; j++) {
      const ResDev &w = j < st->n_integ ? st->integ_res[j] : j < st->n_integ + st->n_main ? st->main_res[j - st->n_integ]
                                                                                          : st->tail_res[j - st->n_integ - st->n_main];
      linear_nk_kernel<<<2 * C / LNK_COLS, 1024, 0, ctx->stream>>>(st->emb.as<float>(), C, n, w.emb_w, 2 * C, w.emb_b, ss_out + (size_t)j * 2 * C,
                                                                 nres * 2 * C, 0);
    }
  };
#ifdef TTS_DEBUG_NO_TIME_GUARD
  mlp(ss_all.as<float>());
  if (false) {
#else
  {
#endif
  const size_t nss = (size_t)n * nres * 2 * C;
  TTS_HIP(ctx, st->ss_chk.reserve(nss * 4 + 4));
  int *flag = (int *)(st->ss_chk.as<float>() + nss);
  bool agreed = false;
  for (int attempt = 0; attempt < 64 && !agreed; attempt++) {
    mlp(ss_all.as<float>());
    mlp(st->ss_chk.as<float>());
    TTS_HIP(ctx, hipMemsetAsync(flag, 0, 4, ctx->stream));
    differ_kernel<<<64, 256, 0, ctx->stream>>>(ss_all.as<unsigned>(), st->ss_chk.as<unsigned>(), nss, flag);
    int h = 1;
    TTS_HIP(ctx, hipMemcpyAsync(&h, flag, 4, hipMemcpyDeviceToHost, ctx->stream));
    TTS_HIP(ctx, hipStreamSynchronize(ctx->stream));
    agreed = h == 0;
    if (!agreed) ctx->time_mlp_retries++;
  }
  if (!agreed) return fail(ctx, TTS_ERR_HIP, "the timestep MLP did not evaluate to the same values twice in 64 attempts");
  }
  TTS_HIP(ctx, hipGetLastError());
  DBG_SUM("time temb", st->temb.p, (size_t)n * C * 4);
  DBG_SUM("time e1", st->e1.p, (size_t)n * C * 4);
  DBG_SUM("time emb", st->emb.p, (size_t)n * C * 4);
  DBG_SUM("time ss_all", ss_all.p, (size_t)n * nres * 2 * C * 4);
  return TTS_OK;
}

static int latent_conditioner(tts_ctx *ctx, DiffState *st, const float *latents_host, const std::vector<int> &lat_lens) {
  Layout &ll = st->lat_lay;
  CHECK(ll.build(ctx, lat_lens));
  Work &wk = st->lat_wk;
  const bool lc_ref = ctx->lc_attn_f32 != 0;
  CHECK(wk.reserve(ctx, ll.rows, ll.ns, lc_ref));
  TTS_HIP(ctx, hipMemsetAsync(wk.X(), 0, (size_t)ll.rows * C * 4, ctx->stream));
  size_t off = 0;
  for (int s = 0; s < ll.ns; s++) {
    TTS_HIP(ctx, hipMemcpyAsync(wk.X() + (size_t)ll.start[s] * C, latents_host + off, (size_t)lat_lens[s] * C * 4,
                                hipMemcpyHostToDevice, ctx->stream));
    off += (size_t)lat_lens[s] * C;
  }
  to_f16_kernel<<<ll.rows, 256, 0, ctx->stream>>>(wk.X(), ll.d_row_seq.as<int>(), wk.A16());
  GemmArgs c3 = gemm_base(ll, wk.A16(), C, 3, C, st->lc_w, C, st->lc_bias);
  c3.mode = GEMM_OUT_F32; c3.outF = wk.X(); c3.ldo = C; c3.resid = nullptr;
  CHECK(gemm(ctx, "diff_gemm", c3, ll));
  for (int i = 0; i < st->n_lc; i++) CHECK(attention_block(ctx, st, ll, wk, wk.X(), st->lc_attn[i], lc_ref));
  CHECK(gn_stats(ctx, ll, wk, wk.X()));
  gn_apply_f32_kernel<<<ll.rows, 256, 0, ctx->stream>>>(wk.X(), ll.d_row_seq.as<int>(), wk.stats.as<float2>(), st->code_g, st->code_b,
                                                        st->mv_tab ? st->mv_tab : st->cond_latent, st->mv_tab ? st->mv_idx : nullptr, wk.H());
  TTS_HIP(ctx, hipGetLastError());
  return TTS_OK;
}

static int network_integrator(tts_ctx *ctx, DiffState *st, Layout &il, Work &iw, float *ce, const float *code_emb, const float *h0, const float *ss) {
  for (int i = 0; i < st->n_integ; i++) {
    if (i == 0) CHECK(res_block(ctx, st, il, iw, ce, st->integ_res[0], ss, code_emb, h0, st->lat ? st->gn_stats_h0.as<long long>() : nullptr));
    else CHECK(res_block(ctx, st, il, iw, ce, st->integ_res[i], ss + (size_t)i * 2 * C));
    CHECK(attention_block(ctx, st, il, iw, ce, st->integ_attn[i]));
  }
  return TTS_OK;
}
static int network_body(tts_ctx *ctx, DiffState *st, Layout &lay, Work &wk, const __half *ce16, const __half *xt16, __half *inp16, float *net, const float *ss) {
  int j = st->n_integ;
  GemmArgs gi = gemm_base(lay, xt16 + XTC, XTC, 3, XTC, st->inp_w, C, st->inp_bias);
  gi.mode = GEMM_OUT_F16; gi.outH = inp16; gi.ldh = C;
  DBG_SUM("ce16", ce16, (size_t)lay.rows * C * 2);
  CHECK(gemm(ctx, "diff_gemm", gi, lay, 0, 300));
  DBG_SUM("inp16", inp16, (size_t)lay.rows * C * 2);
  GemmArgs gc = gemm_base(lay, inp16, C, 2, C, st->integ_w, C, st->integ_bias);
  gc.A[1] = ce16;
  wk.st_x = st->lat ? st->new_stats_slot() : nullptr;
  gc.mode = wk.st_x ? GEMM_OUT_F32_STATS : GEMM_OUT_F32; gc.outF = wk.X(); gc.ldo = C; gc.resid = nullptr;
  gc.st_out = wk.st_x; gc.st_stripe_ll = (int)st->gn_stripe_ll; gc.chunk_seq = lay.d_chunk_seq.as<int>();
  CHECK(gemm(ctx, "diff_gemm", gc, lay));
  DBG_SUM("integ conv", wk.X(), (size_t)lay.rows * C * 4);
  for (int i = 0; i < st->n_main; i++, j++) {
    CHECK(res_block(ctx, st, lay, wk, wk.X(), st->main_res[i], ss + (size_t)j * 2 * C));
    CHECK(attention_block(ctx, st, lay, wk, wk.X(), st->main_attn[i]));
  }
  for (int i = 0; i < st->n_tail; i++, j++) CHECK(res_block(ctx, st, lay, wk, wk.X(), st->tail_res[i], ss + (size_t)j * 2 * C));
  CHECK(gn(ctx, st, lay, wk.X(), st->lat ? wk.st_x : nullptr, st->outn_g, st->outn_b, nullptr, 1, wk.A16()));
  GemmArgs go = gemm_base(lay, wk.A16(), C, 3, C, st->out_w, 256, st->out_bias);
  go.mode = GEMM_OUT_F32; go.outF = net; go.ldo = 256; go.resid = nullptr;
  DBG_SUM("out gn", wk.A16(), (size_t)lay.rows * C * 2);
  CHECK(gemm(ctx, "diff_gemm", go, lay, 200, 0));
  DBG_SUM("net", net, (size_t)lay.rows * 256 * 4);
  return TTS_OK;
}

static int network_forward(tts_ctx *ctx, DiffState *st, StepBufs &sb, const float *ss) {
  Layout &lay = sb.lay;
  Work &wk = sb.wk;
  Layout &il = st->share_integ ? st->ilay : lay;
  Work &iw = st->share_integ ? st->iwk : wk;
  st->gn_site = 0;
  iw.st_x = wk.st_x = iw.st_h = wk.st_h = nullptr;
  if (st->lat) TTS_HIP(ctx, hipMemsetAsync(st->gn_stats.p, 0, (size_t)st->gn_sites_max * st->gn_slot_ll * 8, ctx->stream));
  __half *ce16 = sb.ce16.as<__half>();
  if (st->hoisted) {
    step_row_select_kernel<<<lay.rows, 128, 0, ctx->stream>>>(sb.req, sb.ctr.as<int>(), sb.seq_req, lay.d_row_seq.as<int>(), sb.row_src, (uint4 *)ce16);
  } else {
    float *ce = sb.ce.as<float>();
    if (st->n_integ == 0) TTS_HIP(ctx, hipMemcpyAsync(ce, sb.code_emb.p, (size_t)il.rows * C * 4, hipMemcpyDeviceToDevice, ctx->stream));
    CHECK(network_integrator(ctx, st, il, iw, ce, sb.code_emb.as<float>(), sb.h0.as<float>(), ss));
    if (st->share_integ) gather_f16_kernel<<<lay.rows, 256, 0, ctx->stream>>>(ce, st->ce_src.as<int>(), ce16);
    else to_f16_kernel<<<lay.rows, 256, 0, ctx->stream>>>(ce, lay.d_row_seq.as<int>(), ce16);
  }
  CHECK(network_body(ctx, st, lay, wk, ce16, sb.xt16.as<__half>(), sb.inp16.as<__half>(), sb.net.as<float>(), ss));
  if (st->lat && st->gn_site > st->gn_sites_max) return fail(ctx, TTS_ERR_STATE, "latency_mode: %d statistics slots used, %d reserved", st->gn_site, st->gn_sites_max);
  return TTS_OK;
}

static int precompute_integrator(tts_ctx *ctx, DiffState *st, int n_steps, const float *ss_all, DevBuf &ce16_all) {
  const Layout &lay = st->sb.lay;
  Layout &il = st->share_integ ? st->ilay : st->sb.lay;
  const int per = il.ns, nt_max = std::max(1, 28672 / il.rows);
  const size_t ss_stride = (size_t)st->n_res() * 2 * C;
  TTS_HIP(ctx, ce16_all.reserve((size_t)n_steps * lay.rows * C * 2));
  std::vector<int> il_of_lay(lay.rows, -1), il_seq(il.rows, -1), il_t(il.rows, 0);
  for (int s = 0; s < il.ns; s++)
    for (int t = 0; t < il.len[s]; t++) { il_seq[il.start[s] + t] = s; il_t[il.start[s] + t] = t; }
  if (st->share_integ) il_of_lay = st->ce_src_host;
  else for (int s = 0; s < lay.ns; s++) for (int t = 0; t < lay.len[s]; t++) il_of_lay[lay.start[s] + t] = lay.start[s] + t;
  const bool lat_saved = st->lat;
  st->lat = false;
  int rc = TTS_OK;
  for (int idx0 = 0; idx0 < n_steps && rc == TTS_OK; idx0 += nt_max) {
    const int nt = std::min(nt_max, n_steps - idx0);
    std::vector<int> lens, step_of_seq;
    for (int k = 0; k < nt; k++)
      for (int s = 0; s < per; s++) { lens.push_back(il.len[s]); step_of_seq.push_back(idx0 + k); }
    Layout &pl = st->play;
    if ((rc = pl.build(ctx, lens))) break;
    if ((rc = pl.set_seq_step(ctx, step_of_seq, (int)ss_stride))) break;
    Work &pw = st->pwk;
    if ((rc = pw.reserve(ctx, pl.rows, pl.ns))) break;
    pw.st_x = pw.st_h = nullptr;
    std::vector<int> src(pl.rows, -1), scat((size_t)nt * lay.rows, -1);
    for (int k = 0; k < nt; k++)
      for (int s = 0; s < per; s++)
        for (int t = 0; t < il.len[s]; t++) src[pl.start[k * per + s] + t] = il.start[s] + t;
    for (int k = 0; k < nt; k++)
      for (int r = 0; r < lay.rows; r++) {
        const int ir = il_of_lay[r];
        if (ir >= 0 && il_seq[ir] >= 0) scat[(size_t)k * lay.rows + r] = pl.start[k * per + il_seq[ir]] + il_t[ir];
      }
    TTS_HIP(ctx, st->psrc.reserve(src.size() * 4)); TTS_HIP(ctx, st->pscatter.reserve(scat.size() * 4));
    TTS_HIP(ctx, hipMemcpy(st->psrc.p, src.data(), src.size() * 4, hipMemcpyHostToDevice));
    TTS_HIP(ctx, hipMemcpy(st->pscatter.p, scat.data(), scat.size() * 4, hipMemcpyHostToDevice));
    TTS_HIP(ctx, st->pcode.reserve((size_t)pl.rows * C * 4)); TTS_HIP(ctx, st->ph0.reserve((size_t)pl.rows * C * 4)); TTS_HIP(ctx, st->pce.reserve((size_t)pl.rows * C * 4));
    gather_f32_kernel<<<pl.rows, 256, 0, ctx->stream>>>(st->sb.code_emb.as<float>(), st->psrc.as<int>(), st->pcode.as<float>());
    gather_f32_kernel<<<pl.rows, 256, 0, ctx->stream>>>(st->sb.h0.as<float>(), st->psrc.as<int>(), st->ph0.as<float>());
    float *ce = st->pce.as<float>();
    const float *ssb = ss_all;
    for (int i = 0; i < st->n_integ && rc == TTS_OK; i++) {
      if (i == 0) rc = res_block(ctx, st, pl, pw, ce, st->integ_res[0], ssb, st->pcode.as<float>(), st->ph0.as<float>());
      else rc = res_block(ctx, st, pl, pw, ce, st->integ_res[i], ssb + (size_t)i * 2 * C);
      if (rc == TTS_OK) rc = attention_block(ctx, st, pl, pw, ce, st->integ_attn[i]);
    }
    if (rc) break;
    gather_f16_kernel<<<nt * lay.rows, 256, 0, ctx->stream>>>(ce, st->pscatter.as<int>(), ce16_all.as<__half>() + (size_t)idx0 * lay.rows * C);
    TTS_HIP(ctx, hipGetLastError());
    TTS_HIP(ctx, hipStreamSynchronize(ctx->stream));
  }
  st->lat = lat_saved;
  return rc;
}

static int setup_batch(tts_ctx *ctx, DiffState *st, const float *latents, const std::vector<int> &L, bool cond, bool uncond) {
  const int B = (int)L.size();
  std::vector<int> lens, src;
  if (cond) for (int c = 0; c < B; c++) { lens.push_back(tts_diffusion_frames(L[c])); src.push_back(c); }
  if (uncond) for (int c = 0; c < B; c++) { lens.push_back(tts_diffusion_frames(L[c])); src.push_back(-1); }
  for (int t : lens) if (t < 1) return fail(ctx, TTS_ERR_ARG, "latent too short");
  CHECK(st->sb.lay.build(ctx, lens));
  Layout &lay = st->sb.lay;
  CHECK(st->sb.wk.reserve(ctx, lay.rows, lay.ns));
  CHECK(st->sb.reserve_rows(ctx, (size_t)lay.rows, true));
  TTS_HIP(ctx, hipMemset(st->sb.xt16.p, 0, st->sb.xt16.cap));
  TTS_HIP(ctx, st->seq_src.reserve(lay.ns * 4));
  TTS_HIP(ctx, hipMemcpy(st->seq_src.p, src.data(), lay.ns * 4, hipMemcpyHostToDevice));
  std::vector<int> ilens, isrc, seq_map(lay.ns);
  {
    std::vector<std::pair<int, int>> uniq;
    for (int s = 0; s < lay.ns; s++) {
      int found = -1;
      if (src[s] < 0)
        for (auto &u : uniq) if (u.first == lens[s]) found = u.second;
      if (found < 0) {
        found = (int)ilens.size();
        ilens.push_back(lens[s]); isrc.push_back(src[s]);
        if (src[s] < 0) uniq.push_back({lens[s], found});
      }
      seq_map[s] = found;
    }
  }
  st->share_integ = ctx->share_uncond && (int)ilens.size() < lay.ns;
  if (st->share_integ) {
    CHECK(st->ilay.build(ctx, ilens));
    CHECK(st->iwk.reserve(ctx, st->ilay.rows, st->ilay.ns));
    std::vector<int> cs(lay.rows, -1);
    for (int s = 0; s < lay.ns; s++)
      for (int t = 0; t < lens[s]; t++) cs[lay.start[s] + t] = st->ilay.start[seq_map[s]] + t;
    TTS_HIP(ctx, st->ce_src.reserve((size_t)lay.rows * 4));
    TTS_HIP(ctx, hipMemcpy(st->ce_src.p, cs.data(), (size_t)lay.rows * 4, hipMemcpyHostToDevice));
    st->ce_src_host = cs;
    TTS_HIP(ctx, st->iseq_src.reserve(st->ilay.ns * 4));
    TTS_HIP(ctx, hipMemcpy(st->iseq_src.p, isrc.data(), st->ilay.ns * 4, hipMemcpyHostToDevice));
  }
  Layout &il = st->share_integ ? st->ilay : st->sb.lay;
  if (cond) CHECK(latent_conditioner(ctx, st, latents, L));
  else {
    CHECK(st->lat_lay.build(ctx, L));
    CHECK(st->lat_wk.reserve(ctx, st->lat_lay.rows, st->lat_lay.ns, ctx->lc_attn_f32 != 0));
  }
  build_code_emb_kernel<<<il.rows, 256, 0, ctx->stream>>>(st->lat_wk.H(), st->lat_lay.d_start.as<int>(), st->lat_lay.d_len.as<int>(),
                                                          st->uncond_emb, il.d_row_seq.as<int>(), il.d_row_t.as<int>(), il.d_len.as<int>(),
                                                          (st->share_integ ? st->iseq_src : st->seq_src).as<int>(), st->sb.code_emb.as<float>());
  TTS_HIP(ctx, hipGetLastError());
  st->lat = ctx->latency_mode != 0 && lay.rows <= LAT_MAX_ROWS && il.rows <= LAT_MAX_ROWS;
  if (st->lat) {
    st->gn_stripe_ll = (size_t)std::max(lay.ns, il.ns) * 32 * 4;
    st->gn_slot_ll = st->gn_stripe_ll * FX_STRIPES;
    st->gn_sites_max = 3 * (st->n_integ + st->n_main + st->n_tail) + 2;
    TTS_HIP(ctx, st->gn_stats.reserve((size_t)st->gn_sites_max * st->gn_slot_ll * 8));
    TTS_HIP(ctx, st->gn_stats_h0.reserve(st->gn_slot_ll * 8));
    TTS_HIP(ctx, hipMemsetAsync(st->gn_stats_h0.p, 0, st->gn_slot_ll * 8, ctx->stream));
  }
  if (st->n_integ > 0) {
    TTS_HIP(ctx, reserve_zeroed(st->sb.h0, (size_t)il.rows * C * 4));
    CHECK(res_in_layers(ctx, st, il, st->share_integ ? st->iwk : st->sb.wk, st->sb.code_emb.as<float>(), st->integ_res[0], st->sb.h0.as<float>(), nullptr,
                        st->lat ? st->gn_stats_h0.as<long long>() : nullptr));
  }
  return TTS_OK;
}

static int enqueue_step(tts_ctx *ctx, DiffState *st, StepBufs &sb) {
  Layout &lay = sb.lay;
  const size_t ss_stride = (size_t)st->n_res() * 2 * C;
  int *ctr = sb.ctr.as<int>();
  step_begin_kernel<<<dim3(16, sb.n_live), 256, 0, ctx->stream>>>(sb.req, ctr, sb.live, ss_stride, sb.ss_cur.as<float>());
  step_xt_kernel<<<lay.rows, 128, 0, ctx->stream>>>(sb.req, sb.seq_req, sb.seq_xoff, sb.seq_partner, lay.d_row_seq.as<int>(), lay.d_row_t.as<int>(),
                                                   lay.d_len.as<int>(), sb.xt16.as<__half>() + XTC);
  CHECK(network_forward(ctx, st, sb, sb.ss_cur.as<float>()));
  {
    ProfScope ps(ctx, "diff_update");
    step_update_kernel<<<lay.rows, 128, 0, ctx->stream>>>(sb.net.as<float>(), sb.req, ctr, sb.seq_req, sb.seq_xoff, sb.seq_partner, sb.seq_cand,
                                                         lay.d_row_seq.as<int>(), lay.d_row_t.as<int>(), lay.d_len.as<int>());
  }
  step_advance_kernel<<<(sb.n_live + 63) / 64, 64, 0, ctx->stream>>>(sb.req, ctr, sb.live, sb.n_live);
  TTS_HIP(ctx, hipGetLastError());
  return TTS_OK;
}
static int capture_step(tts_ctx *ctx, DiffState *st, StepBufs &sb) {
  sb.drop_step_graph();
  ctx->capturing = true;
  hipError_t eb = hipStreamBeginCapture(ctx->stream, hipStreamCaptureModeThreadLocal);
  int rc = eb == hipSuccess ? enqueue_step(ctx, st, sb) : TTS_OK;
  hipError_t ee = eb == hipSuccess ? hipStreamEndCapture(ctx->stream, &sb.step_graph) : eb;
  ctx->capturing = false;
  if (rc) return rc;
  TTS_HIP(ctx, ee);
  TTS_HIP(ctx, hipGraphInstantiate(&sb.step_exec, sb.step_graph, nullptr, nullptr, 0));
  return TTS_OK;
}
static bool no_graph_env() {
  static const bool v = getenv("TTS_NO_GRAPH") != nullptr;
  return v;
}

int diff_forward(tts_ctx *ctx, const float *latents, int L, const float *x_t, int timestep, int cond_free, float *out) {
  DiffState *st = ctx->diff;
  if (!st) return fail(ctx, TTS_ERR_STATE, "diffusion model not loaded");
  if (!latents || !x_t || !out || L < 1) return fail(ctx, TTS_ERR_ARG, "tts_diffusion_forward: bad argument");
  std::vector<int> Ls{L};
  CHECK(setup_batch(ctx, st, latents, Ls, !cond_free, cond_free));
  st->hoisted = false;
  StepBufs &sb = st->sb;
  DiffReq &r = st->req;
  const int T = sb.lay.len[0];
  CHECK(precompute_time(ctx, st, std::vector<int>{timestep}, r.ss_all));
  r.n_cand = 1; r.n_steps = 1; r.host_noise = false; r.guided = false; r.sampler = 0;
  r.xoff.assign(1, 0);
  TTS_HIP(ctx, r.x.reserve((size_t)100 * T * 4));
  TTS_HIP(ctx, hipMemcpyAsync(r.x.p, x_t, (size_t)100 * T * 4, hipMemcpyHostToDevice, ctx->stream));
  CHECK(sb.set_single(ctx, r));
  Layout &lay = sb.lay;
  step_xt_kernel<<<lay.rows, 128, 0, ctx->stream>>>(sb.req, sb.seq_req, sb.seq_xoff, sb.seq_partner, lay.d_row_seq.as<int>(), lay.d_row_t.as<int>(),
                                                   lay.d_len.as<int>(), sb.xt16.as<__half>() + XTC);
  CHECK(network_forward(ctx, st, sb, r.ss_all.as<float>()));
  TTS_HIP(ctx, st->out_ct.reserve((size_t)200 * T * 4));
  rows_to_ct_kernel<<<(200 * T + 255) / 256, 256, 0, ctx->stream>>>(sb.net.as<float>(), lay.start[0], T, 200, 256, st->out_ct.as<float>());
  TTS_HIP(ctx, hipMemcpyAsync(out, st->out_ct.p, (size_t)200 * T * 4, hipMemcpyDeviceToHost, ctx->stream));
  TTS_HIP(ctx, hipStreamSynchronize(ctx->stream));
  return TTS_OK;
}

struct ReqSpec {
  const float *latents; const int32_t *rows; int n_cand, n_steps;
  int sampler; double eta; float k;
  bool guided; float temperature;
  const float *voices; int n_voices; const int32_t *voice_of;
  const float *noise; int noise_mode;
  PinnedBuf *stream_noise;
  uint64_t seed; uint32_t stream_base;
  int hoist_max_rows;
  bool timing;
};
static void build_step_tables(const DiffSchedule &sched, int n_steps, bool ddim, bool dpm, bool has_noise, long long total, std::vector<StepEntry> &tab,
                              std::vector<DdimEntry> &dtab, std::vector<DpmEntry> &ptab) {
  tab.assign(n_steps, StepEntry{});
  dtab.assign(ddim ? n_steps : 0, DdimEntry{});
  ptab.assign(dpm ? n_steps : 0, DpmEntry{});
  for (int idx = 0; idx < n_steps; idx++) {
    const int t = n_steps - 1 - idx;
    tab[idx].sc = StepScalars{sched.max_log[t], sched.min_log[t], sched.cfk[t], sched.sqrt_recip[t], sched.sqrt_recipm1[t],
                              sched.coef1[t], sched.coef2[t], t == 0 ? 1 : 0};
    tab[idx].has_noise = has_noise ? 1 : 0;
    tab[idx].noise_off = (long long)(idx + 1) * total;
    tab[idx].philox_step = (unsigned)idx;
    tab[idx].pad = 0;
    if (ddim) dtab[idx] = DdimEntry{sched.c_x0[t], sched.c_eps[t], sched.sigma[t], 0.f};
    if (dpm) ptab[idx] = DpmEntry{sched.dpm_a[t], sched.dpm_b[t], sched.dpm_c[t], sched.dpm_order[t]};
  }
}
static int scale_xT(tts_ctx *ctx, DiffReq &r, float temperature) {
  if (temperature == 1.0f) return TTS_OK;
  scale_xT_kernel<<<(int)((r.total + 255) / 256), 256, 0, ctx->stream>>>(r.x.as<float>(), r.total, temperature);
  TTS_HIP(ctx, hipGetLastError());
  return TTS_OK;
}
static int prepare_request(tts_ctx *ctx, DiffState *st, DiffReq &r, const ReqSpec &sp) {
  const int B = sp.n_cand, n_steps = sp.n_steps;
  struct Reset { DiffState *s; ~Reset() { s->mv_tab = nullptr; s->mv_idx = nullptr; } } reset{st};
  if (sp.voices) {
    const size_t nf = (size_t)sp.n_voices * 2 * C;
    std::vector<float> up(nf + (size_t)B, 0.f);
    memcpy(up.data(), sp.voices, nf * 4);
    if (sp.voice_of) memcpy(up.data() + nf, sp.voice_of, (size_t)B * 4);
    TTS_HIP(ctx, st->mv_buf.reserve(up.size() * 4));
    TTS_HIP(ctx, hipMemcpy(st->mv_buf.p, up.data(), up.size() * 4, hipMemcpyHostToDevice));
    st->mv_tab = st->mv_buf.as<float>();
    st->mv_idx = (const int *)(st->mv_buf.as<float>() + nf);
  }
  CHECK(setup_batch(ctx, st, sp.latents, std::vector<int>(sp.rows, sp.rows + B), true, sp.guided));
  if (sp.timing) (void)hipStreamSynchronize(ctx->stream);
  r.t_setup = std::chrono::steady_clock::now();
  Layout &lay = st->sb.lay;
  r.n_cand = B; r.n_steps = n_steps; r.sampler = sp.sampler; r.seed = sp.seed; r.stream_base = sp.stream_base; r.guided = sp.guided;
  const bool dpm = sp.sampler == 3, ddim = sp.sampler == 1 || dpm;
  const double eta = dpm ? 0.0 : sp.eta;
  const int n_vec = r.n_vec = ddim && eta == 0 ? 1 : n_steps + 1;
  DiffSchedule sched;
  sched.base_k = sp.k;
  sched.build(n_steps);
  if (ddim) sched.build_ddim(eta);
  if (dpm) sched.build_dpmpp();
  std::vector<int> ts(n_steps);
  for (int idx = 0; idx < n_steps; idx++) ts[idx] = sched.timestep_map[n_steps - 1 - idx];
  CHECK(precompute_time(ctx, st, ts, r.ss_all));
  st->hoisted = st->n_integ > 0 && lay.rows <= sp.hoist_max_rows;
  if (st->hoisted) CHECK(precompute_integrator(ctx, st, n_steps, r.ss_all.as<float>(), r.ce16_all));
  r.src_rows = lay.rows;
  r.T.assign(lay.len.begin(), lay.len.begin() + B);
  r.xoff.resize(B);
  r.total = 0;
  for (int c = 0; c < B; c++) { r.xoff[c] = r.total; r.total += (int64_t)100 * lay.len[c]; }
  const int64_t total = r.total;
  TTS_HIP(ctx, r.x.reserve(total * 4));
  if (dpm) TTS_HIP(ctx, r.d_prev.reserve(total * 4));
  r.host_noise = sp.noise != nullptr || sp.noise_mode == TTS_NOISE_REFERENCE;
  r.noise_streamed = r.host_noise && sp.stream_noise != nullptr;
  if (r.noise_streamed && sp.stream_noise->reserve((size_t)total * n_vec * 4) != hipSuccess) { (void)hipGetLastError(); r.noise_streamed = false; }
  if (r.noise_streamed) {
    TTS_HIP(ctx, r.noise.reserve((size_t)total * n_vec * 4));
  } else if (r.host_noise) {
    std::vector<float> hn((size_t)total * n_vec);
    size_t src = 0;
    for (int c = 0; c < B; c++)
      for (int k = 0; k < n_vec; k++) {
        float *dst = hn.data() + (size_t)k * total + r.xoff[c];
        if (sp.noise) {
          memcpy(dst, sp.noise + src, (size_t)100 * lay.len[c] * 4);
          src += (size_t)100 * lay.len[c];
        } else rng_normal_fill(ctx, dst, (int64_t)100 * lay.len[c]);
      }
    TTS_HIP(ctx, r.noise.reserve(hn.size() * 4));
    TTS_HIP(ctx, hipMemcpy(r.noise.p, hn.data(), hn.size() * 4, hipMemcpyHostToDevice));
    TTS_HIP(ctx, hipMemcpyAsync(r.x.p, r.noise.p, total * 4, hipMemcpyDeviceToDevice, ctx->stream));
  } else {
    for (int c = 0; c < B; c++) {
      const int64_t n = (int64_t)100 * lay.len[c];
      philox_fill_kernel<<<(int)((n + 255) / 256), 256, 0, ctx->stream>>>(r.x.as<float>() + r.xoff[c], n, r.seed, r.stream_base + (uint32_t)c, 0xFFFFFFFFu);
    }
    TTS_HIP(ctx, hipGetLastError());
  }
  if (!r.noise_streamed) CHECK(scale_xT(ctx, r, sp.temperature));
  std::vector<StepEntry> tab;
  std::vector<DdimEntry> dtab;
  std::vector<DpmEntry> ptab;
  build_step_tables(sched, n_steps, ddim, dpm, r.host_noise && n_vec > 1, total, tab, dtab, ptab);
  TTS_HIP(ctx, r.tab.reserve(tab.size() * sizeof(StepEntry)));
  TTS_HIP(ctx, hipMemcpyAsync(r.tab.p, tab.data(), tab.size() * sizeof(StepEntry), hipMemcpyHostToDevice, ctx->stream));
  if (ddim) {
    TTS_HIP(ctx, r.dtab.reserve(dtab.size() * sizeof(DdimEntry)));
    TTS_HIP(ctx, hipMemcpyAsync(r.dtab.p, dtab.data(), dtab.size() * sizeof(DdimEntry), hipMemcpyHostToDevice, ctx->stream));
  }
  if (dpm) {
    TTS_HIP(ctx, r.ptab.reserve(ptab.size() * sizeof(DpmEntry)));
    TTS_HIP(ctx, hipMemcpyAsync(r.ptab.p, ptab.data(), ptab.size() * sizeof(DpmEntry), hipMemcpyHostToDevice, ctx->stream));
  }
  TTS_HIP(ctx, hipStreamSynchronize(ctx->stream));
  return TTS_OK;
}

static int diff_sample_with(tts_ctx *ctx, const float *latents, const int32_t *rows, int B, const float *voices, int n_voices, const int32_t *voice_of,
                            int n_steps, const float *noise, int noise_mode, float *mel_out) {
  DiffState *st = ctx->diff;
  static const bool timing = getenv("TTS_TIMING") != nullptr;
  auto now = [] { return std::chrono::steady_clock::now(); };
  auto ms = [](std::chrono::steady_clock::time_point a, std::chrono::steady_clock::time_point b) {
    return std::chrono::duration<double, std::milli>(b - a).count();
  };
  const auto t_begin = now();
  StepBufs &sb = st->sb;
  DiffReq &r = st->req;
  const bool want_pipe = !noise && noise_mode == TTS_NOISE_REFERENCE && B == 1 && ctx->noise_pipeline != 0;
  ReqSpec sp{latents, rows, B, n_steps, ctx->diff_sampler, ctx->ddim_eta, ctx->cond_free_k, ctx->cond_free != 0, (float)ctx->diff_temperature, voices, n_voices, voice_of, noise, noise_mode,
             want_pipe ? &st->noise_host : nullptr, ctx->seed_value, (uint32_t)shard_base(ctx),
             ctx->hoist_integrator == 0 ? 0 : ctx->hoist_integrator > 1 ? ctx->hoist_integrator : HOIST_MAX_ROWS, timing};
  CHECK(prepare_request(ctx, st, r, sp));
  const int64_t total = r.total;
  auto draw_block = [&](int k) {
    float *dst = st->noise_host.as<float>() + (size_t)k * total;
    rng_normal_fill(ctx, dst, total);
    return hipMemcpyAsync(r.noise.as<float>() + (size_t)k * total, dst, (size_t)total * 4, hipMemcpyHostToDevice, ctx->stream);
  };
  if (r.noise_streamed) {
    TTS_HIP(ctx, draw_block(0));
    TTS_HIP(ctx, hipMemcpyAsync(r.x.p, r.noise.p, total * 4, hipMemcpyDeviceToDevice, ctx->stream));
    CHECK(scale_xT(ctx, r, sp.temperature));
  }
  ctx->last_diff_rows = sb.lay.rows; ctx->last_diff_seqs = sb.lay.ns;
  TTS_HIP(ctx, sb.ctr.reserve(64));
  TTS_HIP(ctx, sb.ss_cur.reserve((size_t)st->n_res() * 2 * C * 4));
  TTS_HIP(ctx, hipMemsetAsync(sb.ctr.p, 0, 64, ctx->stream));
  CHECK(sb.set_single(ctx, r));
  if (timing) (void)hipStreamSynchronize(ctx->stream);
  const auto t_pre = now();
  bool prof_diff = ctx->prof_on && ctx->prof_filter.empty();
  for (const std::string &f : ctx->prof_filter) prof_diff |= ctx->prof_on && f.rfind("diff_", 0) == 0;
  const bool use_graph = ctx->diff_graph && !no_graph_env() && n_steps > 2;
  double t_capture = 0;
  if (use_graph) {
    const auto tc0 = now();
    CHECK(capture_step(ctx, st, sb));
    t_capture = ms(tc0, now());
  }
  for (int idx = 0; idx < n_steps; idx++) {
    const bool eager = !use_graph || (prof_diff && idx % ctx->prof_eager_every == 0);
    if (r.noise_streamed && r.n_vec > 1) TTS_HIP(ctx, draw_block(idx + 1));
    if (eager) CHECK(enqueue_step(ctx, st, sb));
    else TTS_HIP(ctx, hipGraphLaunch(sb.step_exec, ctx->stream));
  }
  const auto t_issued = now();
  if (timing) (void)hipStreamSynchronize(ctx->stream);
  const auto t_loop = now();
  TTS_HIP(ctx, hipMemcpyAsync(mel_out, r.x.p, total * 4, hipMemcpyDeviceToHost, ctx->stream));
  TTS_HIP(ctx, hipStreamSynchronize(ctx->stream));
  if (timing)
    fprintf(stderr, "[tts timing] diffusion: setup %.1f ms, time MLP + noise %.1f, %d steps %.1f (issued in %.1f, graph capture + instantiate %.1f), mel copy %.1f\n",
            ms(t_begin, r.t_setup), ms(r.t_setup, t_pre), n_steps, ms(t_pre, t_loop), ms(t_pre, t_issued), t_capture, ms(t_loop, now()));
  return TTS_OK;
}
int diff_sample(tts_ctx *ctx, const float *latents, const int32_t *rows, int B, int n_steps, const float *noise, int noise_mode,
                float *mel_out) {
  if (!ctx->diff) return fail(ctx, TTS_ERR_STATE, "diffusion model not loaded");
  if (!latents || !rows || !mel_out || B < 1 || n_steps < 2) return fail(ctx, TTS_ERR_ARG, "tts_diffusion: bad argument");
  for (int c = 0; c < B; c++) if (rows[c] < 1 || rows[c] > 500) return fail(ctx, TTS_ERR_ARG, "latent rows %d out of range", rows[c]);
  return diff_sample_with(ctx, latents, rows, B, nullptr, 0, nullptr, n_steps, noise, noise_mode, mel_out);
}
int diff_sample_voices(tts_ctx *ctx, const float *latents, const int32_t *rows, int B, const float *voice_latents, int n_voices, const int32_t *voice_of,
                       int n_steps, const float *noise, int noise_mode, float *mel_out) {
  if (!ctx->diff) return fail(ctx, TTS_ERR_STATE, "diffusion model not loaded");
  if (!latents || !rows || !mel_out || B < 1 || n_steps < 2 || !voice_latents || !voice_of) return fail(ctx, TTS_ERR_ARG, "tts_diffusion_multi_voice: bad argument");
  if (n_voices < 1 || n_voices > (1 << 20)) return fail(ctx, TTS_ERR_ARG, "tts_diffusion_multi_voice: %d voices", n_voices);
  for (int c = 0; c < B; c++) {
    if (rows[c] < 1 || rows[c] > 500) return fail(ctx, TTS_ERR_ARG, "latent rows %d out of range", rows[c]);
    if (voice_of[c] < 0 || voice_of[c] >= n_voices)
      return fail(ctx, TTS_ERR_ARG, "tts_diffusion_multi_voice: candidate %d names voice %d of %d", c, voice_of[c], n_voices);
  }
  const size_t nf = (size_t)n_voices * 2 * C;
  for (size_t i = 0; i < nf; i++)
    if (!std::isfinite(voice_latents[i])) return fail(ctx, TTS_ERR_ARG, "tts_diffusion_multi_voice: voice %d holds a non-finite value", (int)(i / (2 * C)));
  return diff_sample_with(ctx, latents, rows, B, voice_latents, n_voices, voice_of, n_steps, noise, noise_mode, mel_out);
}

struct PinnedOptions {
  float gn_eps;
  int ggml_lut, attn_f32, attn_proj_f16, proj_dual_b, gemm_wreg, attn_f32_drop, lc_attn_f32, attn_q64, fp16_check, hoist_integrator, diff_graph, latency_mode, gemm_gn_fuse;
  bool share_uncond;
  static PinnedOptions of(const tts_ctx *c) {
    return PinnedOptions{c->gn_eps, c->ggml_lut, c->attn_f32, c->attn_proj_f16, c->proj_dual_b, c->gemm_wreg, c->attn_f32_drop, c->lc_attn_f32, c->attn_q64,
                         c->fp16_check, c->hoist_integrator, c->diff_graph, c->latency_mode, c->gemm_gn_fuse, c->share_uncond};
  }
  void put(tts_ctx *c) const {
    c->gn_eps = gn_eps; c->ggml_lut = ggml_lut; c->attn_f32 = attn_f32; c->attn_proj_f16 = attn_proj_f16; c->proj_dual_b = proj_dual_b; c->gemm_wreg = gemm_wreg;
    c->attn_f32_drop = attn_f32_drop; c->lc_attn_f32 = lc_attn_f32; c->attn_q64 = attn_q64; c->fp16_check = fp16_check; c->hoist_integrator = hoist_integrator;
    c->diff_graph = diff_graph; c->latency_mode = latency_mode; c->gemm_gn_fuse = gemm_gn_fuse; c->share_uncond = share_uncond;
  }
};
struct DiffSession {
  int max_rows = 0, max_req = 0, buf_rows = 0;
  PinnedOptions pinned{};
  int attn_f32 = 0, hoist = 0, graph = 0, sampler = 0;
  bool share_uncond = true, hoisted = false;
  double eta = 0, temperature = 1.0;
  float k = 2.0f;
  int cond_free = 1;
  std::map<int, std::unique_ptr<DiffReq>> reqs;
  std::vector<char> slot_busy;
  int next_id = 0, captures = 0;
  bool dirty = true;
  StepBufs sb;
};
namespace {
struct SessOptions {
  tts_ctx *c;
  PinnedOptions saved;
  SessOptions(tts_ctx *ctx, const DiffSession &s) : c(ctx), saved(PinnedOptions::of(ctx)) { s.pinned.put(ctx); }
  ~SessOptions() { saved.put(c); }
};
}

void diff_session_close(tts_ctx *ctx) {
  if (!ctx->diff_session) return;
  (void)hipStreamSynchronize(ctx->stream);
  delete ctx->diff_session;
  ctx->diff_session = nullptr;
}
int diff_session_captures(const tts_ctx *ctx) { return ctx->diff_session->captures; }
void diff_session_defaults(const tts_ctx *ctx, tts_diff_request *req) {
  const DiffSession &S = *ctx->diff_session;
  req->sampler = S.sampler; req->ddim_eta = S.eta; req->cond_free_k = S.k;
  if (req->struct_size >= sizeof(tts_diff_request)) { req->temperature = S.temperature; req->cond_free = S.cond_free; }
}
int diff_session_room(const tts_ctx *ctx) {
  const DiffSession &S = *ctx->diff_session;
  int used = 0;
  for (auto &kv : S.reqs) if (!kv.second->finished) used += kv.second->packed;
  return std::max(0, S.max_rows - used);
}

int diff_session_open(tts_ctx *ctx, int max_packed_rows, int max_requests) {
  DiffState *st = ctx->diff;
  if (!st) return fail(ctx, TTS_ERR_STATE, "diffusion model not loaded");
  diff_session_close(ctx);
  std::unique_ptr<DiffSession> s(new DiffSession());
  s->max_rows = max_packed_rows; s->max_req = max_requests; s->buf_rows = (max_packed_rows + 127) & ~127;
  s->attn_f32 = ctx->attn_f32; s->share_uncond = ctx->share_uncond; s->hoist = ctx->hoist_integrator; s->graph = ctx->diff_graph;
  s->pinned = PinnedOptions::of(ctx);
  s->pinned.latency_mode = 0;
  s->sampler = ctx->diff_sampler; s->eta = ctx->ddim_eta; s->k = ctx->cond_free_k; s->temperature = ctx->diff_temperature; s->cond_free = ctx->cond_free;
  s->hoisted = s->hoist != 0 && st->n_integ > 0;
  s->slot_busy.assign((size_t)max_requests, 0);
  const size_t R = (size_t)s->buf_rows;
  StepBufs &sb = s->sb;
  CHECK(sb.wk.reserve(ctx, (int)R, (int)R / 8));
  CHECK(sb.reserve_rows(ctx, R, !s->hoisted));
  if (!s->hoisted) TTS_HIP(ctx, reserve_zeroed(sb.h0, R * C * 4));
  TTS_HIP(ctx, reserve_zeroed(sb.ss_cur, (size_t)max_requests * st->n_res() * 2 * C * 4));
  TTS_HIP(ctx, reserve_zeroed(sb.ctr, (size_t)max_requests * 4));
  ctx->diff_session = s.release();
  return TTS_OK;
}

int diff_session_admit(tts_ctx *ctx, const tts_diff_request *rq) {
  DiffSession &S = *ctx->diff_session;
  DiffState *st = ctx->diff;
  int slot = -1;
  for (int i = 0; i < S.max_req && slot < 0; i++) if (!S.slot_busy[i]) slot = i;
  if (slot < 0) return fail(ctx, TTS_ERR_LIMIT, "tts_diff_session_admit: the session holds %d requests", S.max_req);
  const int B = rq->n_cand;
  const bool grown = rq->struct_size >= sizeof(tts_diff_request);
  const bool guided = (grown ? rq->cond_free : S.cond_free) != 0;
  const float temperature = (float)(grown ? rq->temperature : S.temperature);
  if (S.hoisted) {
    const int cap = S.hoist > 1 ? S.hoist : HOIST_MAX_ROWS, packed = tts_host_diff_packed_rows_ex(rq->rows, B, guided ? 1 : 0);
    if (packed > cap)
      return fail(ctx, TTS_ERR_LIMIT, "tts_diff_session_admit: the request takes %d packed rows; a session opened with hoist_integrator on admits at most %d per request "
                  "(open the session with hoist_integrator 0 for larger ones)", packed, cap);
  }
// ... 147 lines not shown
```

Measured before the change: 143.0.

## Cache time-MLP tables, fuse step-begin kernels, drop host syncs, wreg out head

Caches the per-schedule time-embedding/scale-shift tables across diffusion calls so the time MLP runs only when the timestep schedule or options change. It fuses the per-step ss copy and x_t gather into one kernel with a shared-memory transpose for coalesced loads. Blocking hipMemcpy calls and stream synchronizations in setup become async copies from persistent host buffers. The output-head GEMM gets a register-resident weight path. The async copies from pageable reusable buffers add a lifetime risk if a buffer is reused before its copy completes.

```diff
diff --git a/include/tortoise_mi355x.h b/include/tortoise_mi355x.h
--- a/include/tortoise_mi355x.h
+++ b/include/tortoise_mi355x.h
@@ -184,6 +184,7 @@
                   int n_steps, const float *noise, int noise_mode, float *mel_out);
 int tts_diffusion_last_layout(const tts_ctx *ctx, int32_t *packed_rows_out, int32_t *sequences_out);
 int tts_diffusion_time_mlp_retries(const tts_ctx *ctx);
+int tts_diffusion_time_mlp_evals(const tts_ctx *ctx);
 int tts_diffusion_fp16_check(tts_ctx *ctx, int64_t counts[2]);
 
 int tts_vocoder_samples(int mel_frames);
diff --git a/tortoise.cpp_amd/__init__.py b/tortoise.cpp_amd/__init__.py
--- a/tortoise.cpp_amd/__init__.py
+++ b/tortoise.cpp_amd/__init__.py
@@ -81,7 +81,7 @@
         "tts_ar_begin": (ci, [vp, _i32p, ci, _f32p, ci, ci]), "tts_ar_prefill": (ci, [vp, _f32p]),
         "tts_ar_step": (ci, [vp, _i32p, ci, _f32p]), "tts_ar_latents": (ci, [vp, _i32p, ci, ci, _f32p]),
         "tts_sample": (ci, [vp, _f32p, _i32p, ci, ci, _i32p]),
-        "tts_ar_step_sample": (ci, [vp, _i32p, ci, C.c_uint, _i32p]), "tts_ar_topk_fallbacks": (ci, [vp]), "tts_diffusion_time_mlp_retries": (ci, [vp]), "tts_diffusion_fp16_check": (ci, [vp, C.POINTER(C.c_int64)]),
+        "tts_ar_step_sample": (ci, [vp, _i32p, ci, C.c_uint, _i32p]), "tts_ar_topk_fallbacks": (ci, [vp]), "tts_diffusion_time_mlp_retries": (ci, [vp]), "tts_diffusion_time_mlp_evals": (ci, [vp]), "tts_diffusion_fp16_check": (ci, [vp, C.POINTER(C.c_int64)]),
         "tts_device_numa_node": (ci, [vp, C.c_char_p, ci]), "tts_pin_to_device_numa_node": (ci, [vp]),
         "tts_host_sample_row": (ci, [_f32p, _i32p, ci, cf]), "tts_host_sample_prefiltered": (ci, [_f32p, _i32p, ci, cf, ci]),
         "tts_host_sample_row_ex": (ci, [_f32p, _i32p, ci, cf, cf, ci, cf, cf, ci]), "tts_host_sample_prefiltered_ex": (ci, [_f32p, _i32p, ci, cf, cf, ci, cf, cf, ci, ci]),
@@ -282,6 +282,9 @@
     def time_mlp_retries(self):
         return self.L.tts_diffusion_time_mlp_retries(self.h)
 
+    def time_mlp_evals(self):
+        return self.L.tts_diffusion_time_mlp_evals(self.h)
+
     def ar_latents(self, codes502, n_mel=502):
         codes502 = np.ascontiguousarray(codes502, np.int32).reshape(-1, 502)
         nb = codes502.shape[0]
diff --git a/tortoise.cpp_amd/csrc/api.cpp b/tortoise.cpp_amd/csrc/api.cpp
--- a/tortoise.cpp_amd/csrc/api.cpp
+++ b/tortoise.cpp_amd/csrc/api.cpp
@@ -192,6 +192,8 @@
   else if (k == "proj_dual_b") c->proj_dual_b = value != 0;
   else if (k == "gemm_wreg") c->gemm_wreg = value == 1 ? tts_ctx::GEMM_WREG_ALL : value == 2 ? 1 : value == 3 ? 2 : value == 4 ? 4 : 0;
   else if (k == "gemm_gn_fuse") c->gemm_gn_fuse = value != 0;
+  else if (k == "step_coalesced") c->step_coalesced = value != 0;
+  else if (k == "out_head_wreg") c->out_head_wreg = value != 0;
   else if (k == "lc_attn_f32") c->lc_attn_f32 = value != 0;
   else if (k == "latency_mode") c->latency_mode = value != 0;
   else if (k == "fp16_check") c->fp16_check = value != 0;
@@ -629,6 +631,7 @@
 }
 int tts_ar_topk_fallbacks(const tts_ctx *c) { return c ? c->topk_fallbacks : -1; }
 int tts_diffusion_time_mlp_retries(const tts_ctx *c) { return c ? c->time_mlp_retries : -1; }
+int tts_diffusion_time_mlp_evals(const tts_ctx *c) { return c ? c->time_mlp_evals : -1; }
 int tts_diffusion_fp16_check(tts_ctx *c, int64_t counts[2]) {
   if (!c || !counts) return TTS_ERR_ARG;
   return guarded(c, [&] { return tts::diff_fp16_check(c, counts); });
diff --git a/tortoise.cpp_amd/csrc/common.h b/tortoise.cpp_amd/csrc/common.h
--- a/tortoise.cpp_amd/csrc/common.h
+++ b/tortoise.cpp_amd/csrc/common.h
@@ -141,6 +141,7 @@
   tts::SamplerParams ar_sp;
   int ar_penalty_scope = 0;
   int device_topk = 1;
+  int time_mlp_evals = 0;
   int time_mlp_retries = 0;
   int topk_fallbacks = 0;
   int sampler_threads = -1;
@@ -156,6 +157,8 @@
   int attn_f32 = 0;
   static constexpr int GEMM_WREG_ALL = 7;
   int gemm_wreg = GEMM_WREG_ALL;
+  int step_coalesced = 1;
+  int out_head_wreg = 1;
   int gemm_gn_fuse = 1;
   int proj_dual_b = 1;
   int attn_f32_drop = 0;
diff --git a/tortoise.cpp_amd/csrc/diffusion.hip b/tortoise.cpp_amd/csrc/diffusion.hip
--- a/tortoise.cpp_amd/csrc/diffusion.hip
+++ b/tortoise.cpp_amd/csrc/diffusion.hip
@@ -763,6 +763,64 @@
   }
 }
 
+static constexpr int STEP_ROWS = 32;
+struct StepRow {
+  int slot;
+  int prow;
+  int T, t;
+  long long xo;
+};
+__device__ __forceinline__ StepRow step_row(const ReqDev *__restrict__ req, const int *__restrict__ seq_req, const int64_t *__restrict__ seq_xoff,
+                                            const int *__restrict__ seq_partner, const int *__restrict__ row_seq, const int *__restrict__ row_t,
+                                            const int *__restrict__ seq_len, int r) {
+  StepRow m{-1, -1, 0, 0, 0};
+  const int s = row_seq[r];
+  if (s < 0) return m;
+  const int p = seq_partner[s];
+  if (p < 0) return m;
+  m.slot = seq_req[s];
+  m.T = seq_len[s]; m.t = row_t[r]; m.xo = seq_xoff[s];
+  m.prow = req[m.slot].guided ? p + m.t : -1;
+  return m;
+}
+__global__ __launch_bounds__(256) void step_begin_xt_kernel(const ReqDev *__restrict__ req, const int *__restrict__ ctr, const int *__restrict__ live, int n_live,
+                                                            size_t ss_stride, float *__restrict__ ss_cur, const int *__restrict__ seq_req,
+                                                            const int64_t *__restrict__ seq_xoff, const int *__restrict__ seq_partner,
+                                                            const int *__restrict__ row_seq, const int *__restrict__ row_t, const int *__restrict__ seq_len,
+                                                            __half *__restrict__ xt16) {
+  __shared__ float tile[100][STEP_ROWS + 1];
+  __shared__ StepRow rows[STEP_ROWS];
+  const int r0 = blockIdx.x * STEP_ROWS;
+  if (threadIdx.x < STEP_ROWS) rows[threadIdx.x] = step_row(req, seq_req, seq_xoff, seq_partner, row_seq, row_t, seq_len, r0 + threadIdx.x);
+  for (int b = blockIdx.x; b < 16 * n_live; b += gridDim.x) {
+    const int slot = live[b >> 4], k = ctr[slot];
+    if (k >= req[slot].n_steps) continue;
+    const float4 *src = (const float4 *)(req[slot].ss_all + (size_t)k * ss_stride);
+    float4 *dst = (float4 *)(ss_cur + (size_t)slot * ss_stride);
+    for (size_t i = (size_t)(b & 15) * 256 + threadIdx.x; i < ss_stride / 4; i += (size_t)16 * 256) dst[i] = src[i];
+  }
+  __syncthreads();
+  {
+    const int tx = threadIdx.x & (STEP_ROWS - 1), cy = threadIdx.x / STEP_ROWS;
+    const StepRow m = rows[tx];
+    if (m.slot >= 0) {
+      const float *xs = req[m.slot].x + m.xo + m.t;
+#pragma unroll
+      for (int ch = cy; ch < 100; ch += 256 / STEP_ROWS) tile[ch][tx] = xs[(size_t)ch * m.T];
+    }
+  }
+  __syncthreads();
+  const int lane = threadIdx.x & 63, wave = threadIdx.x >> 6, ch = 2 * lane;
+#pragma unroll
+  for (int j = wave; j < STEP_ROWS; j += 4) {
+    const StepRow m = rows[j];
+    if (m.slot < 0) continue;
+    const __half2 hv = __halves2half2(__float2half_rn(ch < 100 ? tile[ch][j] : 0.f), __float2half_rn(ch + 1 < 100 ? tile[ch + 1][j] : 0.f));
+    *(__half2 *)(xt16 + (size_t)(r0 + j) * XTC + ch) = hv;
+    if (m.prow >= 0) *(__half2 *)(xt16 + (size_t)m.prow * XTC + ch) = hv;
+  }
+}
+
 __global__ void philox_fill_kernel(float *__restrict__ x, int64_t n, uint64_t seed, uint32_t stream, uint32_t step) {
   int64_t i = (int64_t)blockIdx.x * blockDim.x + threadIdx.x;
   if (i < n) x[i] = philox_normal(seed, stream, step, (uint32_t)i);
@@ -899,14 +957,18 @@
   int64_t total = 0;
   DevBuf ce16_all;
   DevBuf code_emb, h0;
-  DevBuf ss_all, tab, dtab, ptab, x, d_prev, noise;
+  std::shared_ptr<DevBuf> ss_all;
+  DevBuf tab, dtab, ptab, x, d_prev, noise;
+  std::vector<StepEntry> h_tab;
+  std::vector<DdimEntry> h_dtab;
+  std::vector<DpmEntry> h_ptab;
   std::chrono::steady_clock::time_point t_setup;
   int id = 0, slot = 0, done = 0, cls = 0, packed = 0;
   bool finished = false;
   std::vector<int> seq_src;
   int src_rows = 0;
   ReqDev dev() const {
-    return ReqDev{ss_all.as<float>(), tab.as<StepEntry>(), dtab.as<DdimEntry>(), sampler == 3 ? ptab.as<DpmEntry>() : nullptr, ce16_all.as<__half>(), x.as<float>(),
+    return ReqDev{ss_all ? ss_all->as<float>() : nullptr, tab.as<StepEntry>(), dtab.as<DdimEntry>(), sampler == 3 ? ptab.as<DpmEntry>() : nullptr, ce16_all.as<__half>(), x.as<float>(),
                   sampler == 3 ? d_prev.as<float>() : nullptr, host_noise ? noise.as<float>() : nullptr, seed, n_steps, sampler, src_rows, stream_base, guided ? 1 : 0};
   }
 };
@@ -916,6 +978,7 @@
   Work wk;
   DevBuf code_emb, h0, ce, ce16, inp16, xt16, net;
   DevBuf ss_cur, ctr;
+  std::vector<char> tables_host;
   DevBuf tables;
   const ReqDev *req = nullptr;
   const int64_t *seq_xoff = nullptr;
@@ -942,13 +1005,14 @@
   }
   int set_tables(tts_ctx *ctx, const std::vector<ReqDev> &reqs, const std::vector<int> &slots, const std::vector<int64_t> &xoff, const std::vector<int> &sreq,
                  const std::vector<int> &partner, const std::vector<int> &cand, const std::vector<int> &rsrc) {
-    std::vector<char> img;
+    std::vector<char> &img = tables_host;
+    img.clear();
     auto put = [&](const void *p, size_t bytes) { const size_t o = img.size(); img.insert(img.end(), (const char *)p, (const char *)p + bytes); return o; };
     const size_t o_req = put(reqs.data(), reqs.size() * sizeof(ReqDev)), o_xoff = put(xoff.data(), xoff.size() * 8);
     const size_t o_sreq = put(sreq.data(), sreq.size() * 4), o_partner = put(partner.data(), partner.size() * 4), o_cand = put(cand.data(), cand.size() * 4);
     const size_t o_rsrc = put(rsrc.data(), rsrc.size() * 4), o_live = put(slots.data(), slots.size() * 4);
     TTS_HIP(ctx, tables.reserve(img.size()));
-    TTS_HIP(ctx, hipMemcpy(tables.p, img.data(), img.size(), hipMemcpyHostToDevice));
+    TTS_HIP(ctx, hipMemcpyAsync(tables.p, img.data(), img.size(), hipMemcpyHostToDevice, ctx->stream));
     const char *b = tables.as<char>();
     req = (const ReqDev *)(b + o_req); seq_xoff = (const int64_t *)(b + o_xoff);
     seq_req = (const int *)(b + o_sreq); seq_partner = (const int *)(b + o_partner); seq_cand = (const int *)(b + o_cand);
@@ -978,6 +1042,7 @@
   float *te0_w = nullptr, *te0_b = nullptr, *te2_w = nullptr, *te2_b = nullptr;
   float *inp_bias = nullptr, *integ_bias = nullptr, *outn_g = nullptr, *outn_b = nullptr, *out_bias = nullptr;
   __half *lc_w = nullptr, *inp_w = nullptr, *integ_w = nullptr, *out_w = nullptr;
+  __half *out_wf = nullptr;
   std::vector<void *> owned;
   StepBufs sb;
   DiffReq req;
@@ -996,6 +1061,14 @@
   size_t gn_slot_ll = 0, gn_stripe_ll = 0;
   long long *new_stats_slot() { long long *p = gn_stats.as<long long>() + (size_t)gn_site * gn_slot_ll; gn_site++; return p; }
   DevBuf temb, e1, emb, ss_chk, seq_src, lat_in16, out_ct;
+  struct TimeCache {
+    bool valid = false;
+    std::vector<int> ts;
+    int n_res = 0, act = 0, sampler = 0, attn_f32 = 0;
+    std::shared_ptr<DevBuf> ss;
+    std::vector<float> te;
+  } tcache;
+  std::vector<float> mv_host;
   PinnedBuf noise_host;
   DevBuf mv_buf;
   const float *mv_tab = nullptr;
@@ -1164,7 +1237,7 @@
   }
   for (int i = 0; i < st->n_tail; i++) jobs.emplace_back([&ld, S, i]() { return ld.res("layers." + std::to_string(S->n_main + i), S->tail_res[i]); });
   J(ld.f32("out.0.weight", C, &S->outn_g)); J(ld.f32("out.0.bias", C, &S->outn_b));
-  J(ld.conv16("out.2.weight", 200, C, 3, 256, C, &S->out_w));
+  J(ld.conv16("out.2.weight", 200, C, 3, 256, C, &S->out_w, &S->out_wf));
   jobs.emplace_back([&ld, S]() -> int {
     const HostTensor *t = ld.get("out.2.bias", 200);
     if (!t) return TTS_ERR_FORMAT;
@@ -1703,15 +1776,25 @@
     if (a[i] != b[i]) *flag = 1;
 }
 
-static int precompute_time(tts_ctx *ctx, DiffState *st, const std::vector<int> &timesteps, DevBuf &ss_all) {
+static int precompute_time(tts_ctx *ctx, DiffState *st, const std::vector<int> &timesteps, int sampler, std::shared_ptr<DevBuf> &ss_out) {
   const int n = (int)timesteps.size(), nres = st->n_res();
-  std::vector<float> te((size_t)n * C);
+  const int act = ctx->ggml_lut ? 2 : 1;
+  DiffState::TimeCache &tc = st->tcache;
+  if (tc.valid && tc.ts == timesteps && tc.n_res == nres && tc.act == act && tc.sampler == sampler && tc.attn_f32 == ctx->attn_f32) {
+    ss_out = tc.ss;
+    return TTS_OK;
+  }
+  tc.valid = false;
+  ss_out.reset();
+  if (!tc.ss || tc.ss.use_count() > 1) tc.ss = std::make_shared<DevBuf>();
+  DevBuf &ss_all = *tc.ss;
+  ctx->time_mlp_evals++;
+  std::vector<float> &te = tc.te;
+  te.resize((size_t)n * C);
   for (int i = 0; i < n; i++) timestep_embedding(timesteps[i], te.data() + (size_t)i * C);
   TTS_HIP(ctx, st->temb.reserve(te.size() * 4)); TTS_HIP(ctx, st->e1.reserve(te.size() * 4)); TTS_HIP(ctx, st->emb.reserve(te.size() * 4));
   TTS_HIP(ctx, ss_all.reserve((size_t)n * nres * 2 * C * 4));
   TTS_HIP(ctx, hipMemcpyAsync(st->temb.p, te.data(), te.size() * 4, hipMemcpyHostToDevice, ctx->stream));
-  TTS_HIP(ctx, hipStreamSynchronize(ctx->stream));
-  const int act = ctx->ggml_lut ? 2 : 1;
   auto mlp = [&](float *ss_out) {
     linear_nk_kernel<<<C / LNK_COLS, 1024, 0, ctx->stream>>>(st->temb.as<float>(), C, n, st->te0_w, C, st->te0_b, st->e1.as<float>(), C, act);
     linear_nk_kernel<<<C / LNK_COLS, 1024, 0, ctx->stream>>>(st->e1.as<float>(), C, n, st->te2_w, C, st->te2_b, st->emb.as<float>(), C, act);
@@ -1750,6 +1833,9 @@
   DBG_SUM("time e1", st->e1.p, (size_t)n * C * 4);
   DBG_SUM("time emb", st->emb.p, (size_t)n * C * 4);
   DBG_SUM("time ss_all", ss_all.p, (size_t)n * nres * 2 * C * 4);
+  tc.ts = timesteps; tc.n_res = nres; tc.act = act; tc.sampler = sampler; tc.attn_f32 = ctx->attn_f32;
+  tc.valid = true;
+  ss_out = tc.ss;
   return TTS_OK;
 }
 
@@ -1808,6 +1894,7 @@
   CHECK(gn(ctx, st, lay, wk.X(), st->lat ? wk.st_x : nullptr, st->outn_g, st->outn_b, nullptr, 1, wk.A16()));
   GemmArgs go = gemm_base(lay, wk.A16(), C, 3, C, st->out_w, 256, st->out_bias);
   go.mode = GEMM_OUT_F32; go.outF = net; go.ldo = 256; go.resid = nullptr;
+  if (ctx->out_head_wreg && gemm_auto_th(lay.rows, 256) >= 4) { go.Wf = st->out_wf; go.wreg = 1; go.th = 8; }
   DBG_SUM("out gn", wk.A16(), (size_t)lay.rows * C * 2);
   CHECK(gemm(ctx, "diff_gemm", go, lay, 200, 0));
   DBG_SUM("net", net, (size_t)lay.rows * 256 * 4);
@@ -1965,9 +2052,15 @@
   Layout &lay = sb.lay;
   const size_t ss_stride = (size_t)st->n_res() * 2 * C;
   int *ctr = sb.ctr.as<int>();
-  step_begin_kernel<<<dim3(16, sb.n_live), 256, 0, ctx->stream>>>(sb.req, ctr, sb.live, ss_stride, sb.ss_cur.as<float>());
-  step_xt_kernel<<<lay.rows, 128, 0, ctx->stream>>>(sb.req, sb.seq_req, sb.seq_xoff, sb.seq_partner, lay.d_row_seq.as<int>(), lay.d_row_t.as<int>(),
-                                                   lay.d_len.as<int>(), sb.xt16.as<__half>() + XTC);
+  if (ctx->step_coalesced) {
+    step_begin_xt_kernel<<<lay.rows / STEP_ROWS, 256, 0, ctx->stream>>>(sb.req, ctr, sb.live, sb.n_live, ss_stride, sb.ss_cur.as<float>(), sb.seq_req, sb.seq_xoff,
+                                                                      sb.seq_partner, lay.d_row_seq.as<int>(), lay.d_row_t.as<int>(), lay.d_len.as<int>(),
+                                                                      sb.xt16.as<__half>() + XTC);
+  } else {
+    step_begin_kernel<<<dim3(16, sb.n_live), 256, 0, ctx->stream>>>(sb.req, ctr, sb.live, ss_stride, sb.ss_cur.as<float>());
+    step_xt_kernel<<<lay.rows, 128, 0, ctx->stream>>>(sb.req, sb.seq_req, sb.seq_xoff, sb.seq_partner, lay.d_row_seq.as<int>(), lay.d_row_t.as<int>(),
+                                                     lay.d_len.as<int>(), sb.xt16.as<__half>() + XTC);
+  }
   CHECK(network_forward(ctx, st, sb, sb.ss_cur.as<float>()));
   {
     ProfScope ps(ctx, "diff_update");
@@ -2005,7 +2098,7 @@
   StepBufs &sb = st->sb;
   DiffReq &r = st->req;
   const int T = sb.lay.len[0];
-  CHECK(precompute_time(ctx, st, std::vector<int>{timestep}, r.ss_all));
+  CHECK(precompute_time(ctx, st, std::vector<int>{timestep}, 0, r.ss_all));
   r.n_cand = 1; r.n_steps = 1; r.host_noise = false; r.guided = false; r.sampler = 0;
   r.xoff.assign(1, 0);
   TTS_HIP(ctx, r.x.reserve((size_t)100 * T * 4));
@@ -2014,7 +2107,7 @@
   Layout &lay = sb.lay;
   step_xt_kernel<<<lay.rows, 128, 0, ctx->stream>>>(sb.req, sb.seq_req, sb.seq_xoff, sb.seq_partner, lay.d_row_seq.as<int>(), lay.d_row_t.as<int>(),
                                                    lay.d_len.as<int>(), sb.xt16.as<__half>() + XTC);
-  CHECK(network_forward(ctx, st, sb, r.ss_all.as<float>()));
+  CHECK(network_forward(ctx, st, sb, r.ss_all->as<float>()));
   TTS_HIP(ctx, st->out_ct.reserve((size_t)200 * T * 4));
   rows_to_ct_kernel<<<(200 * T + 255) / 256, 256, 0, ctx->stream>>>(sb.net.as<float>(), lay.start[0], T, 200, 256, st->out_ct.as<float>());
   TTS_HIP(ctx, hipMemcpyAsync(out, st->out_ct.p, (size_t)200 * T * 4, hipMemcpyDeviceToHost, ctx->stream));
@@ -2061,11 +2154,12 @@
   struct Reset { DiffState *s; ~Reset() { s->mv_tab = nullptr; s->mv_idx = nullptr; } } reset{st};
   if (sp.voices) {
     const size_t nf = (size_t)sp.n_voices * 2 * C;
-    std::vector<float> up(nf + (size_t)B, 0.f);
+    std::vector<float> &up = st->mv_host;
+    up.assign(nf + (size_t)B, 0.f);
     memcpy(up.data(), sp.voices, nf * 4);
     if (sp.voice_of) memcpy(up.data() + nf, sp.voice_of, (size_t)B * 4);
     TTS_HIP(ctx, st->mv_buf.reserve(up.size() * 4));
-    TTS_HIP(ctx, hipMemcpy(st->mv_buf.p, up.data(), up.size() * 4, hipMemcpyHostToDevice));
+    TTS_HIP(ctx, hipMemcpyAsync(st->mv_buf.p, up.data(), up.size() * 4, hipMemcpyHostToDevice, ctx->stream));
     st->mv_tab = st->mv_buf.as<float>();
     st->mv_idx = (const int *)(st->mv_buf.as<float>() + nf);
   }
@@ -2084,9 +2178,9 @@
   if (dpm) sched.build_dpmpp();
   std::vector<int> ts(n_steps);
   for (int idx = 0; idx < n_steps; idx++) ts[idx] = sched.timestep_map[n_steps - 1 - idx];
-  CHECK(precompute_time(ctx, st, ts, r.ss_all));
+  CHECK(precompute_time(ctx, st, ts, sp.sampler, r.ss_all));
   st->hoisted = st->n_integ > 0 && lay.rows <= sp.hoist_max_rows;
-  if (st->hoisted) CHECK(precompute_integrator(ctx, st, n_steps, r.ss_all.as<float>(), r.ce16_all));
+  if (st->hoisted) CHECK(precompute_integrator(ctx, st, n_steps, r.ss_all->as<float>(), r.ce16_all));
   r.src_rows = lay.rows;
   r.T.assign(lay.len.begin(), lay.len.begin() + B);
   r.xoff.resize(B);
@@ -2122,9 +2216,9 @@
     TTS_HIP(ctx, hipGetLastError());
   }
   if (!r.noise_streamed) CHECK(scale_xT(ctx, r, sp.temperature));
-  std::vector<StepEntry> tab;
-  std::vector<DdimEntry> dtab;
-  std::vector<DpmEntry> ptab;
+  std::vector<StepEntry> &tab = r.h_tab;
+  std::vector<DdimEntry> &dtab = r.h_dtab;
+  std::vector<DpmEntry> &ptab = r.h_ptab;
   build_step_tables(sched, n_steps, ddim, dpm, r.host_noise && n_vec > 1, total, tab, dtab, ptab);
   TTS_HIP(ctx, r.tab.reserve(tab.size() * sizeof(StepEntry)));
   TTS_HIP(ctx, hipMemcpyAsync(r.tab.p, tab.data(), tab.size() * sizeof(StepEntry), hipMemcpyHostToDevice, ctx->stream));
@@ -2136,7 +2230,6 @@
     TTS_HIP(ctx, r.ptab.reserve(ptab.size() * sizeof(DpmEntry)));
     TTS_HIP(ctx, hipMemcpyAsync(r.ptab.p, ptab.data(), ptab.size() * sizeof(DpmEntry), hipMemcpyHostToDevice, ctx->stream));
   }
-  TTS_HIP(ctx, hipStreamSynchronize(ctx->stream));
   return TTS_OK;
 }
 
@@ -2224,16 +2317,16 @@
 
 struct PinnedOptions {
   float gn_eps;
-  int ggml_lut, attn_f32, attn_proj_f16, proj_dual_b, gemm_wreg, attn_f32_drop, lc_attn_f32, attn_q64, fp16_check, hoist_integrator, diff_graph, latency_mode, gemm_gn_fuse;
+  int ggml_lut, attn_f32, attn_proj_f16, proj_dual_b, gemm_wreg, attn_f32_drop, lc_attn_f32, attn_q64, fp16_check, hoist_integrator, diff_graph, latency_mode, gemm_gn_fuse, step_coalesced, out_head_wreg;
   bool share_uncond;
   static PinnedOptions of(const tts_ctx *c) {
     return PinnedOptions{c->gn_eps, c->ggml_lut, c->attn_f32, c->attn_proj_f16, c->proj_dual_b, c->gemm_wreg, c->attn_f32_drop, c->lc_attn_f32, c->attn_q64,
-                         c->fp16_check, c->hoist_integrator, c->diff_graph, c->latency_mode, c->gemm_gn_fuse, c->share_uncond};
+                         c->fp16_check, c->hoist_integrator, c->diff_graph, c->latency_mode, c->gemm_gn_fuse, c->step_coalesced, c->out_head_wreg, c->share_uncond};
   }
   void put(tts_ctx *c) const {
     c->gn_eps = gn_eps; c->ggml_lut = ggml_lut; c->attn_f32 = attn_f32; c->attn_proj_f16 = attn_proj_f16; c->proj_dual_b = proj_dual_b; c->gemm_wreg = gemm_wreg;
     c->attn_f32_drop = attn_f32_drop; c->lc_attn_f32 = lc_attn_f32; c->attn_q64 = attn_q64; c->fp16_check = fp16_check; c->hoist_integrator = hoist_integrator;
-    c->diff_graph = diff_graph; c->latency_mode = latency_mode; c->gemm_gn_fuse = gemm_gn_fuse; c->share_uncond = share_uncond;
+    c->diff_graph = diff_graph; c->latency_mode = latency_mode; c->gemm_gn_fuse = gemm_gn_fuse; c->step_coalesced = step_coalesced; c->out_head_wreg = out_head_wreg; c->share_uncond = share_uncond;
   }
 };
 struct DiffSession {
```

Result: no change. 143.9 (median of 6 runs) (+0.6%).
